# verlab/accelerated_features

Measured on NVIDIA B200. Metric: image-pairs/sec (extract+match) VGA batch=64, higher is better.
Workload: dtype f32

## Files before the change

### accelerated_features_b200/_lib.py

```python
from __future__ import annotations

import ctypes as C
import os

_HERE = os.path.dirname(os.path.abspath(__file__))
LIB_PATH = os.path.join(_HERE, "libxfeat_sm100.so")
_lib = None
ABI_VERSION = 2
N_OVERFLOW = -1

c_i, c_f, c_p, c_sz, c_i64 = C.c_int, C.c_float, C.c_void_p, C.c_size_t, C.c_int64

SIGNATURES = {
    "xfeat_abi_version": (c_i, []),
    "xfeat_last_error": (C.c_char_p, []),
    "xfeat_launch_count": (C.c_ulonglong, []),
    "xfeat_packed_weight_floats": (c_sz, []),
    "xfeat_create": (c_i, [C.POINTER(c_p), c_i, c_p, c_sz]),
    "xfeat_destroy": (None, [c_p]),
    "xfeat_resize_bilinear": (c_i, [c_p, c_i, c_i, c_i, c_i, c_i, c_i64, c_i64, c_i64, c_i64, c_i, c_p, c_i, c_i, c_f, c_f, c_p]),
    "xfeat_preprocess": (c_i, [c_p, c_i, c_i, c_i, c_i, c_i, c_i64, c_i64, c_i64, c_i64, c_i, c_i, c_i, c_p, c_p, c_p]),
    "xfeat_preprocess_scaled": (c_i, [c_p, c_i, c_i, c_i, c_i, c_i, c_i64, c_i64, c_i64, c_i64, c_i, c_i, c_i, c_f, c_f, c_p, c_p, c_p]),
    "xfeat_set_conv_impl": (None, [c_i]),
    "xfeat_set_halo_desc_mode": (None, [c_i]),
    "xfeat_get_conv_impl": (c_i, []),
    "xfeat_set_block1_fused": (None, [c_i]),
    "xfeat_get_block1_fused": (c_i, []),
    "xfeat_net_workspace_bytes": (c_sz, [c_i, c_i, c_i]),
    "xfeat_net": (c_i, [c_p, c_p, c_i, c_i, c_i, c_p, c_p, c_p, c_p, c_p, c_sz, c_p]),
    "xfeat_sparse_workspace_bytes": (c_sz, [c_i, c_i, c_i, c_i]),
    "xfeat_detect_sparse": (c_i, [c_p, c_p, c_p, c_p, c_i, c_i, c_i, c_i, c_f, c_f, c_f, c_p, c_p, c_p, c_p, c_p, c_p, c_p, c_sz, c_p]),
    "xfeat_detect_sparse_split": (c_i, [c_p, c_p, c_p, c_p, c_i, c_i, c_i, c_i, c_f, c_f, c_f, c_p, c_p, c_p, c_p, c_p, c_p, c_p, c_i, c_p, c_sz, c_p]),
    "xfeat_dense_workspace_bytes": (c_sz, [c_i, c_i, c_i, c_i]),
    "xfeat_detect_dense": (c_i, [c_p, c_p, c_p, c_i, c_i, c_i, c_i, c_f, c_f, c_f, c_f, c_i, c_i, c_p, c_p, c_p, c_p, c_p, c_sz, c_p]),
    "xfeat_set_mnn_impl": (None, [c_i]),
    "xfeat_get_mnn_impl": (c_i, []),
    "xfeat_mnn_workspace_bytes": (c_sz, [c_i, c_i, c_i]),
    "xfeat_mnn_match": (c_i, [c_p, c_p, c_i, c_i64, c_p, c_p, c_i, c_i64, c_i, c_f, c_p, c_p, c_p, c_p, c_sz, c_p]),
    "xfeat_mnn_match_bounded": (c_i, [c_p, c_p, c_i, c_i64, c_p, c_p, c_i, c_i64, c_i, c_f, c_f, c_p, c_p, c_p, c_p, c_sz, c_p]),
    "xfeat_mnn_presplit_workspace_bytes": (c_sz, [c_i, c_i, c_i]),
    "xfeat_mnn_match_presplit": (c_i, [c_p, c_p, c_i, c_p, c_p, c_i, c_i, c_i, c_i, c_f, c_p, c_p, c_p, c_p, c_sz, c_p]),
    "xfeat_gather_matches": (c_i, [c_p, c_p, c_i, c_i, c_p, c_p, c_p, c_i, c_p, c_p, c_p]),
    "xfeat_refine_workspace_bytes": (c_sz, [c_i, c_i]),
    "xfeat_refine": (c_i, [c_p, c_p, c_p, c_p, c_p, c_p, c_p, c_p, c_p, c_i, c_i, c_i, c_f, c_p, c_p, c_p, c_sz, c_p]),
    "xfeat_kpts_heatmap": (c_i, [c_p, c_i, c_i, c_i, c_f, c_p, c_p]),
    "xfeat_nms_workspace_bytes": (c_sz, [c_i, c_i, c_i]),
    "xfeat_nms_count": (c_i, [c_p, c_i, c_i, c_i, c_i, c_f, c_p, c_p, c_sz, c_p]),
    "xfeat_nms_write": (c_i, [c_p, c_i, c_i, c_i, c_i, c_f, c_p, c_i, c_p, c_sz, c_p]),
    "xfeat_interpolate_sparse": (c_i, [c_p, c_p, c_i, c_i, c_i, c_i, c_i, c_i, c_i, c_i, c_p, c_p]),
    "xfeat_subpix_softmax2d": (c_i, [c_p, c_i64, c_f, c_p, c_p]),
    "xfeat_fine_matcher_workspace_bytes": (c_sz, [c_i]),
    "xfeat_fine_matcher": (c_i, [c_p, c_p, c_i, c_p, c_p, c_sz, c_p]),
    "xfeat_ransac_workspace_bytes": (c_sz, [c_i, c_i]),
    "xfeat_ransac_homography": (c_i, [c_p, c_p, c_p, c_i, c_i, c_f, c_i, C.c_uint32, c_p, c_p, c_p, c_p, c_sz, c_p]),
    "xfeat_ransac_essential": (c_i, [c_p, c_p, c_p, c_i, c_i, c_f, c_i, C.c_uint32, c_p, c_p, c_p, c_p, c_sz, c_p]),
    "xfeat_debug_conv_layer": (c_i, [c_p, c_i, c_p, c_i, c_i, c_i, c_p, c_p]),
    "xfeat_debug_conv_layer_tc": (c_i, [c_p, c_i, c_p, c_i, c_i, c_i, c_p, c_p, c_sz, c_p]),
    "xfeat_debug_block1_tail": (c_i, [c_p, c_p, c_p, c_i, c_i, c_i, c_p, c_p, c_sz, c_p]),
}


class XFeatLibraryError(RuntimeError):
    pass


def load():
    global _lib
    if _lib is not None:
        return _lib
    if not os.path.exists(LIB_PATH):
        raise XFeatLibraryError(
            f"{LIB_PATH} not found: build it with `python -m accelerated_features_b200.build` "
            "(there is no CPU / PyTorch fallback for the XFeat hot path)")
    lib = C.CDLL(LIB_PATH)
    for name, (res, args) in SIGNATURES.items():
        fn = getattr(lib, name)
        fn.restype = res
        fn.argtypes = args
    if lib.xfeat_abi_version() != ABI_VERSION:
        raise XFeatLibraryError(f"ABI version mismatch: library {lib.xfeat_abi_version()} != binding {ABI_VERSION}")
    _lib = lib
    return lib


def check(rc: int, what: str = ""):
    if rc != 0:
        msg = load().xfeat_last_error().decode(errors="replace")
        raise XFeatLibraryError(f"{what} failed (code {rc}): {msg}")
```

### accelerated_features_b200/csrc/api.cu

```cuda
#include <stdarg.h>

#include <map>
#include <mutex>
#include <utility>
#include <vector>

#include "common.cuh"

namespace xf {

static thread_local char g_err[1024] = "";
unsigned long long g_launches = 0;
int g_conv_impl = 2;

int ensure_dyn_smem(const void* func, size_t bytes) {
  static std::mutex mu;
  static std::map<std::pair<int, const void*>, size_t> done;
  int dev = 0;
  XF_CUDA(cudaGetDevice(&dev));
  std::lock_guard<std::mutex> lock(mu);
  size_t& cur = done[std::make_pair(dev, func)];
  if (bytes > cur) {
    XF_CUDA(cudaFuncSetAttribute(func, cudaFuncAttributeMaxDynamicSharedMemorySize, (int)bytes));
    cur = bytes;
  }
  return XF_OK;
}

void set_error(const char* fmt, ...) {
  va_list ap;
  va_start(ap, fmt);
  vsnprintf(g_err, sizeof(g_err), fmt, ap);
  va_end(ap);
}

struct NetWs {
  float *a1, *a2, *a3, *x1s, *t4a, *x2;
  float *t8a, *t8b, *x3, *fin, *f1, *f2;
  float *t16a, *t16b, *x4;
  float *t32a, *t32b, *x5;
};

static void carve_net(Bump& bump, int B, int H, int W, NetWs& ws) {
  const size_t p1 = (size_t)B * H * W, p2 = p1 / 4, p4 = p1 / 16, p8 = p1 / 64, p16 = p1 / 256, p32 = p1 / 1024;
  ws.a1 = bump.take<float>(p1 * 4);
  ws.a2 = bump.take<float>(p2 * 8);
  ws.a3 = bump.take<float>(p2 * 8);
  ws.x1s = bump.take<float>(p4 * 32);
  ws.t4a = bump.take<float>(p4 * 32);
  ws.x2 = bump.take<float>(p4 * 32);
  ws.t8a = bump.take<float>(p8 * 64);
  ws.t8b = bump.take<float>(p8 * 64);
  ws.x3 = bump.take<float>(p8 * 64);
  ws.fin = bump.take<float>(p8 * 64);
  ws.f1 = bump.take<float>(p8 * 64);
  ws.f2 = bump.take<float>(p8 * 64);
  ws.t16a = bump.take<float>(p16 * 64);
  ws.t16b = bump.take<float>(p16 * 64);
  ws.x4 = bump.take<float>(p16 * 64);
  ws.t32a = bump.take<float>(p32 * 128);
  ws.t32b = bump.take<float>(p32 * 128);
  ws.x5 = bump.take<float>(p32 * 64);
}

}

extern "C" int xfeat_abi_version(void) { return XFEAT_ABI_VERSION; }
extern "C" const char* xfeat_last_error(void) { return xf::g_err; }
extern "C" unsigned long long xfeat_launch_count(void) { return xf::g_launches; }
extern "C" size_t xfeat_packed_weight_floats(void) { return xf::make_layer_table().total; }

extern "C" int xfeat_create(xfeat_ctx** out, int device, const float* packed_host, size_t n_floats) {
  XF_REQUIRE(out && packed_host, "create: null pointer");
  const xf::LayerTable t = xf::make_layer_table();
  XF_REQUIRE(n_floats == t.total, "create: packed blob has %zu floats, expected %zu", n_floats, t.total);
  xf::DeviceGuard guard(device);
  XF_REQUIRE(guard.ok, "create: cudaSetDevice(%d) failed", device);
  cudaDeviceProp prop;
  XF_CUDA(cudaGetDeviceProperties(&prop, device));
  if (prop.major != 10) {
    xf::set_error("create: device %d is sm_%d%d; this library contains sm_100a code only", device, prop.major, prop.minor);
    return XF_E_UNSUPPORTED;
  }
  xfeat_ctx* c = new xfeat_ctx();
  c->device = device;
  c->sm_count = prop.multiProcessorCount;
  c->table = t;
  c->h_weights = (float*)malloc(sizeof(float) * t.total);
  memcpy(c->h_weights, packed_host, sizeof(float) * t.total);
  c->d_weights = nullptr;
  cudaError_t e = cudaMalloc(&c->d_weights, sizeof(float) * t.total);
  if (e == cudaSuccess) e = cudaMemcpy(c->d_weights, packed_host, sizeof(float) * t.total, cudaMemcpyHostToDevice);
  if (e != cudaSuccess) {
    xf::set_error("create: weight upload failed: %s", cudaGetErrorString(e));
    if (c->d_weights) cudaFree(c->d_weights);
    free(c->h_weights);
    delete c;
    return XF_E_CUDA;
  }
  c->d_tcw = nullptr;
  c->d_mlpw = nullptr;
  int rc = xf::conv_tc_prepare(c);
  if (rc == XF_OK) rc = xf::mlp_tc_prepare(c);
  if (rc != XF_OK) {
    cudaFree(c->d_weights);
    if (c->d_tcw) cudaFree(c->d_tcw);
    if (c->d_mlpw) cudaFree(c->d_mlpw);
    free(c->h_weights);
    delete c;
    return rc;
  }
  *out = c;
  return XF_OK;
}

extern "C" void xfeat_set_conv_impl(int impl) { xf::g_conv_impl = (impl < 0 || impl > 2) ? 1 : impl; }
extern "C" int xfeat_get_conv_impl(void) { return xf::g_conv_impl; }

extern "C" void xfeat_destroy(xfeat_ctx* ctx) {
  if (!ctx) return;
  xf::DeviceGuard guard(ctx->device);
  if (ctx->d_weights) cudaFree(ctx->d_weights);
  if (ctx->d_tcw) cudaFree(ctx->d_tcw);
  if (ctx->d_mlpw) cudaFree(ctx->d_mlpw);
  free(ctx->h_weights);
  delete ctx;
}

extern "C" size_t xfeat_net_workspace_bytes(int B, int H, int W) {
  xf::Bump bump(nullptr, 0);
  xf::NetWs ws;
  xf::carve_net(bump, B, H, W, ws);
  return bump.used();
}

extern "C" int xfeat_net(xfeat_ctx* ctx, const float* d_xn, int B, int H, int W, float* d_feats, float* d_heat,
                         float* d_reliability, float* d_kpt_logits, void* d_ws, size_t ws_bytes, void* stream) {
  using namespace xf;
  XF_REQUIRE(ctx && d_xn && d_feats && d_heat && d_reliability && d_ws, "net: null pointer");
  XF_REQUIRE(B > 0 && B <= 65535 && H > 0 && W > 0 && H % 32 == 0 && W % 32 == 0, "net: bad shape B=%d H=%d W=%d", B, H, W);
  XF_CUDA(cudaSetDevice(ctx->device));
  cudaStream_t st = (cudaStream_t)stream;
  Bump bump(d_ws, ws_bytes);
  NetWs ws;
  carve_net(bump, B, H, W, ws);
  if (!bump.ok) {
    set_error("net: workspace too small (%zu < %zu)", ws_bytes, bump.used());
    return XF_E_WORKSPACE;
  }
  const int H4 = H / 4, W4 = W / 4, H8 = H / 8, W8 = W / 8, H16 = H / 16, W16 = W / 16, H32 = H / 32, W32 = W / 32;
  int rc;
#define XF_RUN(call) \
  if ((rc = (call)) != XF_OK) return rc
  if (g_conv_impl == 0) {
    XF_RUN(launch_stem_chain(ctx->h_weights, ctx->table, d_xn, ws.a1, ws.a2, ws.a3, ws.x1s, nullptr, B, H, W, st));
    XF_RUN(launch_conv_layer(ctx, L_B2_0, ws.x1s, IN_NHWC, B, H4, W4, ws.t4a, st));
    XF_RUN(launch_conv_layer(ctx, L_B2_1, ws.t4a, IN_NHWC, B, H4, W4, ws.x2, st));
    XF_RUN(launch_conv_layer(ctx, L_B3_0, ws.x2, IN_NHWC, B, H4, W4, ws.t8a, st));
    XF_RUN(launch_conv_layer(ctx, L_B3_1, ws.t8a, IN_NHWC, B, H8, W8, ws.t8b, st));
    XF_RUN(launch_conv_layer(ctx, L_B3_2, ws.t8b, IN_NHWC, B, H8, W8, ws.x3, st));
    XF_RUN(launch_conv_layer(ctx, L_B4_0, ws.x3, IN_NHWC, B, H8, W8, ws.t16a, st));
    XF_RUN(launch_conv_layer(ctx, L_B4_1, ws.t16a, IN_NHWC, B, H16, W16, ws.t16b, st));
    XF_RUN(launch_conv_layer(ctx, L_B4_2, ws.t16b, IN_NHWC, B, H16, W16, ws.x4, st));
    XF_RUN(launch_conv_layer(ctx, L_B5_0, ws.x4, IN_NHWC, B, H16, W16, ws.t32a, st));
  } else {
    __half *s4a = (__half*)ws.x1s, *s4b = (__half*)ws.t4a, *s4c = (__half*)ws.x2;
    __half *s8a = (__half*)ws.t8a, *s8b = (__half*)ws.t8b, *s16a = (__half*)ws.t16a, *s16b = (__half*)ws.t16b;
    if (g_conv_impl == 2) {
      XF_RUN(launch_stem_chain(ctx->h_weights, ctx->table, d_xn, ws.a1, ws.a2, ws.a3, nullptr, nullptr, B, H, W, st, 1));
      XF_RUN(launch_block1_tail(ctx, (const __half*)ws.a2, d_xn, B, H4, W4, (__half*)ws.a3, s4a, nullptr, st));
    } else {
      XF_RUN(launch_stem_chain(ctx->h_weights, ctx->table, d_xn, ws.a1, ws.a2, ws.a3, nullptr, s4a, B, H, W, st));
    }
    XF_RUN(launch_conv_tc(ctx, L_B2_0, s4a, B, H4, W4, s4b, nullptr, st));
    XF_RUN(launch_conv_tc(ctx, L_B2_1, s4b, B, H4, W4, s4c, nullptr, st));
    XF_RUN(launch_conv_tc(ctx, L_B3_0, s4c, B, H4, W4, s8a, nullptr, st));
    XF_RUN(launch_conv_tc(ctx, L_B3_1, s8a, B, H8, W8, s8b, nullptr, st));
    XF_RUN(launch_conv_tc(ctx, L_B3_2, s8b, B, H8, W8, s8a, nullptr, st));
    XF_RUN(launch_conv_tc(ctx, L_B4_0, s8a, B, H8, W8, s16a, nullptr, st));
    XF_RUN(launch_conv_tc(ctx, L_B4_1, s16a, B, H16, W16, s16b, nullptr, st));
    XF_RUN(launch_conv_tc(ctx, L_B4_2, s16b, B, H16, W16, s16a, nullptr, st));
    __half *s32a = (__half*)ws.t32a, *s32b = (__half*)ws.t32b;
    XF_RUN(launch_conv_tc(ctx, L_B5_0, s16a, B, H16, W16, s32a, nullptr, st));
    XF_RUN(launch_conv_tc(ctx, L_B5_1, s32a, B, H32, W32, s32b, nullptr, st));
    XF_RUN(launch_conv_tc(ctx, L_B5_2, s32b, B, H32, W32, s32a, nullptr, st));
    XF_RUN(launch_conv_tc(ctx, L_B5_3, s32a, B, H32, W32, s32b, nullptr, st));
  }
  if (g_conv_impl == 0) {
    XF_RUN(launch_conv_layer(ctx, L_B5_1, ws.t32a, IN_NHWC, B, H32, W32, ws.t32b, st));
    XF_RUN(launch_conv_layer(ctx, L_B5_2, ws.t32b, IN_NHWC, B, H32, W32, ws.t32a, st));
    XF_RUN(launch_conv_layer(ctx, L_B5_3, ws.t32a, IN_NHWC, B, H32, W32, ws.x5, st));
  }
  if (g_conv_impl == 0) {
    XF_RUN(launch_fuse_pyramid(ws.x3, ws.x4, ws.x5, ws.fin, nullptr, B, H8, W8, st));
    XF_RUN(launch_conv_layer(ctx, L_FU_0, ws.fin, IN_NHWC, B, H8, W8, ws.f1, st));
    XF_RUN(launch_conv_layer(ctx, L_FU_1, ws.f1, IN_NHWC, B, H8, W8, ws.f2, st));
    XF_RUN(launch_conv_layer(ctx, L_FU_2, ws.f2, IN_NHWC, B, H8, W8, d_feats, st));
    XF_RUN(launch_conv_layer(ctx, L_HH_0, d_feats, IN_NHWC, B, H8, W8, ws.t8a, st));
    XF_RUN(launch_conv_layer(ctx, L_HH_1, ws.t8a, IN_NHWC, B, H8, W8, ws.t8b, st));
    XF_RUN(launch_reliability(ctx, ws.t8b, d_reliability, (int64_t)B * H8 * W8, st));
    XF_RUN(launch_conv_layer(ctx, L_KH_0, d_xn, IN_UNFOLD8, B, H8, W8, ws.t8a, st));
    XF_RUN(launch_conv_layer(ctx, L_KH_1, ws.t8a, IN_NHWC, B, H8, W8, ws.t8b, st));
    XF_RUN(launch_conv_layer(ctx, L_KH_2, ws.t8b, IN_NHWC, B, H8, W8, ws.t8a, st));
    XF_RUN(launch_kpt_softmax(ctx, ws.t8a, d_heat, d_kpt_logits, B, H8, W8, st));
  } else {
    __half *s8a = (__half*)ws.t8a, *s8b = (__half*)ws.t8b, *sfin = (__half*)ws.fin, *sf1 = (__half*)ws.f1, *sf2 = (__half*)ws.f2;
    XF_RUN(launch_fuse_pyramid_split(s8a, (const __half*)ws.t16a, (const __half*)ws.t32b, sfin, B, H8, W8, st));
    XF_RUN(launch_conv_tc(ctx, L_FU_0, sfin, B, H8, W8, sf1, nullptr, st));
    XF_RUN(launch_conv_tc(ctx, L_FU_1, sf1, B, H8, W8, sf2, nullptr, st));
    XF_RUN(launch_conv_tc(ctx, L_FU_2, sf2, B, H8, W8, s8a, d_feats, st));
    if (g_conv_impl == 2) {
      XF_RUN(launch_head_chain(ctx, 1, s8a, B, H8, W8, d_reliability, nullptr, st));
      XF_RUN(launch_head_chain(ctx, 0, d_xn, B, H8, W8, d_heat, d_kpt_logits, st));
      return XF_OK;
    }
    XF_RUN(launch_conv_tc(ctx, L_HH_0, s8a, B, H8, W8, s8b, nullptr, st));
    XF_RUN(launch_conv_tc(ctx, L_HH_1, s8b, B, H8, W8, nullptr, ws.t8a, st));
    XF_RUN(launch_reliability(ctx, ws.t8a, d_reliability, (int64_t)B * H8 * W8, st));
    XF_RUN(launch_unfold8_split(d_xn, s8b, B, H8, W8, st));
    XF_RUN(launch_conv_tc(ctx, L_KH_0, s8b, B, H8, W8, s8a, nullptr, st));
    XF_RUN(launch_conv_tc(ctx, L_KH_1, s8a, B, H8, W8, s8b, nullptr, st));
    XF_RUN(launch_conv_tc(ctx, L_KH_2, s8b, B, H8, W8, nullptr, ws.t8a, st));
    XF_RUN(launch_kpt_softmax(ctx, ws.t8a, d_heat, d_kpt_logits, B, H8, W8, st));
  }
#undef XF_RUN
  return XF_OK;
}
```

### accelerated_features_b200/csrc/block1_tc.cu

```cuda
#include <cuda_fp16.h>

#include <stdlib.h>

#include "common.cuh"
#include "tc_common.cuh"

namespace xf {

constexpr int B1_THREADS = 448;
constexpr int B1_NP = 4;
constexpr int B1_W2_BYTES = 9 * 2 * 8 * 32;
constexpr int B1_W3_BYTES = 9 * 2 * 32 * 32;
constexpr int B1_W_PAD = 23 * 1024;
constexpr int B1_PB_MAX = 30 * 1024;
constexpr int B1_PLANE_MAX = 6 * 1024;

struct Block1Params {
  CUtensorMap amap;
  CUtensorMap w2map;
  CUtensorMap w3map;
  const float* bias2;
  const float* bias3;
  const float* skip_w;
  const float* xn;
  float inv_ws2, inv_ws3;
  int B, H4, W4;
  int TQH, TQW, PW2, PQW, M2;
  int PB, PLB;
  int tmem_cols;
  __half* out_split;
  float* out_f32;
  FastDiv div_img, div_x;
};

__global__ void __launch_bounds__(B1_THREADS, 1) block1_tc_kernel(const __grid_constant__ Block1Params P) {
  extern __shared__ unsigned char smem_raw[];
  unsigned char* base = reinterpret_cast<unsigned char*>(((uintptr_t)smem_raw + 1023) & ~(uintptr_t)1023);
  unsigned char* sW2 = base;
  unsigned char* sW3 = sW2 + B1_W2_BYTES;
  unsigned char* sP = base + B1_W_PAD;
  unsigned char* sQ = sP + (size_t)B1_NP * P.PB;
  uint64_t* bars = reinterpret_cast<uint64_t*>(sQ + (size_t)8 * P.PLB);
  uint64_t* w_full = bars;
  uint64_t* p_full = bars + 1;
  uint64_t* p_empty = p_full + B1_NP;
  uint64_t* acc2_full = p_empty + B1_NP;
  uint64_t* acc2_empty = acc2_full + 2;
  uint64_t* q_full = acc2_empty + 2;
  uint64_t* q_empty = q_full + 2;
  uint64_t* acc3_full = q_empty + 2;
  uint64_t* acc3_empty = acc3_full + 2;
  uint32_t* tmem_slot = reinterpret_cast<uint32_t*>(acc3_empty + 2);
  float* sB2 = reinterpret_cast<float*>(tmem_slot + 2);
  float* sB3 = sB2 + 8;
  float* sSkip = sB3 + 32;

  const int warp = threadIdx.x >> 5, lane = threadIdx.x & 31;
  const int tiles_x = (P.W4 + P.TQW - 1) / P.TQW, tiles_y = (P.H4 + P.TQH - 1) / P.TQH;
  const int tiles_img = tiles_x * tiles_y;
  const int n_tiles = tiles_img * P.B;
  const int H2 = 2 * P.H4, W2 = 2 * P.W4;
  const int ACC2 = P.M2 * 16;
  const uint32_t acc3_col = 2u * ACC2;

  if (threadIdx.x < 8) sB2[threadIdx.x] = __ldg(P.bias2 + threadIdx.x);
  if (threadIdx.x < 32) sB3[threadIdx.x] = threadIdx.x < 24 ? __ldg(P.bias3 + threadIdx.x) : 0.f;
  if (threadIdx.x < 64) {
    const int c = threadIdx.x % 32, wb = threadIdx.x / 32;
    sSkip[threadIdx.x] = c < 24 ? __ldg(P.skip_w + wb * 24 + c) : 0.f;
  }
  if (warp == 0 && lane == 0) {
    tc::tma_prefetch_desc(&P.amap);
    tc::tma_prefetch_desc(&P.w2map);
    tc::tma_prefetch_desc(&P.w3map);
    tc::mbar_init(w_full, 1);
    for (int i = 0; i < B1_NP; ++i) {
      tc::mbar_init(&p_full[i], 1);
      tc::mbar_init(&p_empty[i], 1);
    }
    for (int i = 0; i < 2; ++i) {
      tc::mbar_init(&acc2_full[i], 1);
      tc::mbar_init(&acc2_empty[i], 8);
      tc::mbar_init(&q_full[i], 8);
      tc::mbar_init(&q_empty[i], 1);
      tc::mbar_init(&acc3_full[i], 1);
      tc::mbar_init(&acc3_empty[i], 4);
    }
    tc::fence_barrier_init();
  }
  if (warp == 1) {
    tc::tmem_alloc(tmem_slot, P.tmem_cols);
    tc::tmem_relinquish();
  }
  tc::tc_fence_before();
  __syncthreads();
  tc::tc_fence_after();
  const uint32_t tmem = *tmem_slot;

  if (warp == 0) {
    if (tc::elect_one()) {
      tc::mbar_expect_tx(w_full, (uint32_t)(B1_W2_BYTES + B1_W3_BYTES));
      for (int i = 0; i < 18; ++i) tc::tma_load_2d(sW2 + i * 256, &P.w2map, w_full, 0, i * 8);
      for (int i = 0; i < 18; ++i) tc::tma_load_2d(sW3 + i * 1024, &P.w3map, w_full, 0, i * 32);
      const uint32_t patch_tx = (uint32_t)(2 * P.TQH + 3) * P.PW2 * 32;
      uint32_t tcount = 0;
      for (int tile = blockIdx.x; tile < n_tiles; tile += gridDim.x, ++tcount) {
        const int b = (int)fdiv((unsigned)tile, P.div_img), rem = tile - b * tiles_img;
        const int ty_ = (int)fdiv((unsigned)rem, P.div_x), tx_ = rem - ty_ * tiles_x;
        const int s = tcount % B1_NP;
        tc::mbar_wait(&p_empty[s], ((tcount / B1_NP) & 1) ^ 1);
        tc::mbar_expect_tx(&p_full[s], patch_tx);
        tc::tma_load_4d(sP + (size_t)s * P.PB, &P.amap, &p_full[s], 0, 2 * tx_ * P.TQW - 2, 2 * ty_ * P.TQH - 2, b);
      }
    }
    __syncwarp();
  } else if (warp == 1) {
    if (tc::elect_one()) {
      constexpr uint32_t idesc2 = tc::make_idesc( 0, 128, 16);
      constexpr uint32_t idesc3 = tc::make_idesc( 0, 128, 64);
      tc::mbar_wait(w_full, 0);
      const uint32_t w2_base = tc::smem_u32(sW2), w3_base = tc::smem_u32(sW3);
      const uint32_t p_base = tc::smem_u32(sP), q_base = tc::smem_u32(sQ);
      const int n_mine = n_tiles > (int)blockIdx.x ? (n_tiles - 1 - (int)blockIdx.x) / (int)gridDim.x + 1 : 0;
      for (int t = 0; t <= n_mine; ++t) {
        if (t < n_mine) {
          const int s = t % B1_NP, a = t & 1;
          tc::mbar_wait(&acc2_empty[a], ((t >> 1) & 1) ^ 1);
          tc::mbar_wait(&p_full[s], (t / B1_NP) & 1);
          tc::tc_fence_after();
          const uint32_t pb = p_base + (uint32_t)s * P.PB;
          for (int mt = 0; mt < P.M2; ++mt) {
            const uint32_t d = tmem + (uint32_t)(a * ACC2 + mt * 16);
            for (int tap = 0; tap < 9; ++tap) {
              const uint32_t row = (uint32_t)(mt * 128 + (tap / 3) * P.PW2 + (tap % 3));
              tc::umma_f16(d, tc::make_desc_sw32(pb + row * 32u, 256), tc::make_desc_sw32(w2_base + tap * 512u, 256), idesc2,
                           tap ? 1u : 0u);
            }
          }
          tc::umma_commit(&p_empty[s]);
          tc::umma_commit(&acc2_full[a]);
        }
        if (t > 0) {
          const int u = t - 1, a = u & 1;
          tc::mbar_wait(&acc3_empty[a], ((u >> 1) & 1) ^ 1);
          tc::mbar_wait(&q_full[a], (u >> 1) & 1);
          tc::tc_fence_after();
          const uint32_t qb = q_base + (uint32_t)a * 4u * P.PLB;
          const uint32_t d = tmem + acc3_col + (uint32_t)a * 64u;
          for (int tap = 0; tap < 9; ++tap) {
            const int ky = tap / 3, kx = tap % 3;
            const uint32_t addr = qb + (uint32_t)((ky & 1) * 2 + (kx & 1)) * P.PLB + (uint32_t)((ky >> 1) * P.PQW + (kx >> 1)) * 32u;
            tc::umma_f16(d, tc::make_desc_sw32(addr, 256), tc::make_desc_sw32(w3_base + tap * 2048u, 256), idesc3, tap ? 1u : 0u);
          }
          tc::umma_commit(&q_empty[a]);
          tc::umma_commit(&acc3_full[a]);
        }
      }
    }
    __syncwarp();
  } else if (warp < 10) {
    const int q = warp & 3, eg = (warp - 2) >> 2;
    const int hmax = 2 * P.TQH + 1, wmax = 2 * P.TQW + 1;
    uint32_t tcount = 0;
    for (int tile = blockIdx.x; tile < n_tiles; tile += gridDim.x, ++tcount) {
      const int a = tcount & 1;
      const int b = (int)fdiv((unsigned)tile, P.div_img), rem = tile - b * tiles_img;
      const int ty_ = (int)fdiv((unsigned)rem, P.div_x), tx_ = rem - ty_ * tiles_x;
      const int y0 = 2 * ty_ * P.TQH - 1, x0 = 2 * tx_ * P.TQW - 1;
      unsigned char* qb = sQ + (size_t)a * 4 * P.PLB;
      tc::mbar_wait(&acc2_full[a], (tcount >> 1) & 1);
      tc::mbar_wait(&q_empty[a], ((tcount >> 1) & 1) ^ 1);
      tc::tc_fence_after();
      for (int mt = eg; mt < P.M2; mt += 2) {
        uint32_t v[16];
        __syncwarp();
        tc::tmem_ld_32x16(tmem + ((uint32_t)(q * 32) << 16) + (uint32_t)(a * ACC2 + mt * 16), v);
        tc::tmem_ld_wait();
        const int m = mt * 128 + q * 32 + lane;
        const int h = m / P.PW2, w = m - h * P.PW2;
        if (h < hmax && w < wmax) {
          const int y = y0 + h, x = x0 + w;
          uint32_t hw[4] = {0u, 0u, 0u, 0u}, lw[4] = {0u, 0u, 0u, 0u};
          if (y >= 0 && y < H2 && x >= 0 && x < W2) {
            float o[8];
#pragma unroll
            for (int c = 0; c < 8; ++c) o[c] = fmaxf(fmaf(__uint_as_float(v[c]) + __uint_as_float(v[8 + c]), P.inv_ws2, sB2[c]), 0.f);
#pragma unroll
            for (int j = 0; j < 4; ++j) {
              const __half2 hh = __floats2half2_rn(o[2 * j], o[2 * j + 1]);
              const float2 hf = __half22float2(hh);
              const __half2 ll = __floats2half2_rn(o[2 * j] - hf.x, o[2 * j + 1] - hf.y);
              hw[j] = *reinterpret_cast<const uint32_t*>(&hh);
              lw[j] = *reinterpret_cast<const uint32_t*>(&ll);
            }
          }
          const int r = (h >> 1) * P.PQW + (w >> 1);
          unsigned char* rp = qb + (size_t)((h & 1) * 2 + (w & 1)) * P.PLB + r * 32;
          const int sw = (r >> 2) & 1;
          *reinterpret_cast<uint4*>(rp + (sw << 4)) = make_uint4(hw[0], hw[1], hw[2], hw[3]);
          *reinterpret_cast<uint4*>(rp + ((sw ^ 1) << 4)) = make_uint4(lw[0], lw[1], lw[2], lw[3]);
        }
      }
      tc::fence_proxy_async();
      tc::tc_fence_before();
      __syncwarp();
      if (lane == 0) {
        tc::mbar_arrive(&acc2_empty[a]);
        tc::mbar_arrive(&q_full[a]);
      }
    }
  } else {
    const int q = warp & 3;
    const int m = q * 32 + lane;
    const int i = m / P.PQW, j = m - i * P.PQW;
    const bool lane_ok = (i < P.TQH) && (j < P.TQW);
    const int W0 = P.W4 * 4;
    auto fetch_xn = [&](int tile, float4 (&xv)[4]) {
      if (tile >= n_tiles) return;
      const int b = (int)fdiv((unsigned)tile, P.div_img), rem = tile - b * tiles_img;
      const int ty_ = (int)fdiv((unsigned)rem, P.div_x), tx_ = rem - ty_ * tiles_x;
      const int y = ty_ * P.TQH + i, x = tx_ * P.TQW + j;
      if (lane_ok && y < P.H4 && x < P.W4) {
        const float* xp = P.xn + ((int64_t)b * P.H4 * 4 + y * 4) * W0 + x * 4;
#pragma unroll
        for (int rr = 0; rr < 4; ++rr) xv[rr] = __ldg(reinterpret_cast<const float4*>(xp + (int64_t)rr * W0));
      }
    };
    float4 xv[4] = {};
    fetch_xn(blockIdx.x, xv);
    uint32_t tcount = 0;
    for (int tile = blockIdx.x; tile < n_tiles; tile += gridDim.x, ++tcount) {
      const int a = tcount & 1;
      const int b = (int)fdiv((unsigned)tile, P.div_img), rem = tile - b * tiles_img;
      const int ty_ = (int)fdiv((unsigned)rem, P.div_x), tx_ = rem - ty_ * tiles_x;
      const int y = ty_ * P.TQH + i, x = tx_ * P.TQW + j;
      float4 xnext[4] = {};
      fetch_xn(tile + (int)gridDim.x, xnext);
      tc::mbar_wait(&acc3_full[a], (tcount >> 1) & 1);
      tc::tc_fence_after();
      uint32_t v[64];
      __syncwarp();
#pragma unroll
      for (int c = 0; c < 2; ++c) {
        uint32_t t[32];
        tc::tmem_ld_32x32(tmem + ((uint32_t)(q * 32) << 16) + acc3_col + (uint32_t)a * 64u + c * 32, t);
#pragma unroll
        for (int k = 0; k < 32; ++k) v[c * 32 + k] = t[k];
      }
      tc::tmem_ld_wait();
      tc::tc_fence_before();
      __syncwarp();
      if (lane == 0) tc::mbar_arrive(&acc3_empty[a]);
      if (lane_ok && y < P.H4 && x < P.W4) {
        const int64_t pix = ((int64_t)b * P.H4 + y) * P.W4 + x;
        float o[32];
#pragma unroll
        for (int c = 0; c < 32; ++c) o[c] = fmaxf(fmaf(__uint_as_float(v[c]) + __uint_as_float(v[32 + c]), P.inv_ws3, sB3[c]), 0.f);
        float sacc = 0.f;
#pragma unroll
        for (int rr = 0; rr < 4; ++rr) {
          sacc += xv[rr].x; sacc += xv[rr].y; sacc += xv[rr].z; sacc += xv[rr].w;
        }
        const float skipv = sacc * (1.0f / 16.0f);
#pragma unroll
        for (int c = 0; c < 32; ++c) o[c] += fmaf(skipv, sSkip[c], sSkip[32 + c]);
        if (P.out_f32) tc::store_f32_row<32>(P.out_f32 + pix * 24, o, 24);
        if (P.out_split) {
          __half* hp = P.out_split + pix * 64;
          tc::store_split_row<32>(hp, hp + 32, o);
        }
      }
#pragma unroll
      for (int rr = 0; rr < 4; ++rr) xv[rr] = xnext[rr];
    }
  }
  tc::tc_fence_before();
  __syncthreads();
  if (warp == 1) {
    tc::tc_fence_after();
    tc::tmem_dealloc(tmem, P.tmem_cols);
  }
}

struct Block1Tile { int TQH, TQW, M2; };

static Block1Tile pick_block1_tile(int H4, int W4) {
  Block1Tile best = {0, 0, 0};
  double best_cost = 1e30;
  for (int tqw = 4; tqw <= 62; ++tqw) {
    const int pqw = tqw + 1, pw2 = 2 * tqw + 3;
    for (int tqh = 1; tqh * pqw <= 128; ++tqh) {
      const int m2 = cdiv((2 * tqh + 1) * pw2, 128);
      if ((m2 * 128 + 2 * pw2 + 2) * 32 > B1_PB_MAX || (128 + pqw + 1) * 32 > B1_PLANE_MAX) continue;
      const double tiles = (double)cdiv(W4, tqw) * cdiv(H4, tqh);
      const double cost = tiles * ((m2 + 1) * 128.0 + 0.15 * (2 * tqh + 3) * pw2);
      if (cost < best_cost) { best_cost = cost; best = {tqh, tqw, m2}; }
    }
  }
  return best;
}

int g_block1_fused = 1;

static bool block1_fused() {
  static const bool unfused = getenv("XFEAT_BLOCK1_UNFUSED") != nullptr;
  return g_block1_fused && !unfused;
}

static int launch_block1_fused(const xfeat_ctx* ctx, const __half* a2_split, const float* xn, int B, int H4, int W4,
                               __half* out_split, float* out_f32, cudaStream_t st) {
  PFN_encodeTiled enc = get_encode_tiled();
  if (!enc) {
    set_error("cuTensorMapEncodeTiled entry point not available");
    return XF_E_CUDA;
  }
  const Block1Tile tl = pick_block1_tile(H4, W4);
  Block1Params P;
  P.TQH = tl.TQH; P.TQW = tl.TQW; P.M2 = tl.M2;
  P.PW2 = 2 * tl.TQW + 3;
  P.PQW = tl.TQW + 1;
  P.PB = (int)align_up((size_t)(tl.M2 * 128 + 2 * P.PW2 + 2) * 32, 1024);
  P.PLB = (int)align_up((size_t)(128 + P.PQW + 1) * 32, 1024);
  int cols = 32;
  while (cols < 2 * tl.M2 * 16 + 128) cols *= 2;
  P.tmem_cols = cols;
  const int H2 = 2 * H4, W2 = 2 * W4;
  const cuuint64_t dims[4] = {16, (cuuint64_t)W2, (cuuint64_t)H2, (cuuint64_t)B};
  const cuuint64_t strides[3] = {32, (cuuint64_t)W2 * 32, (cuuint64_t)H2 * W2 * 32};
  const cuuint32_t box[4] = {16, (cuuint32_t)P.PW2, (cuuint32_t)(2 * P.TQH + 3), 1};
  const cuuint32_t estr[4] = {1, 1, 1, 1};
  CUresult r = enc(&P.amap, CU_TENSOR_MAP_DATA_TYPE_FLOAT16, 4, (void*)a2_split, dims, strides, box, estr,
                   CU_TENSOR_MAP_INTERLEAVE_NONE, CU_TENSOR_MAP_SWIZZLE_32B, CU_TENSOR_MAP_L2_PROMOTION_L2_256B,
                   CU_TENSOR_MAP_FLOAT_OOB_FILL_NONE);
  if (r != CUDA_SUCCESS) {
    set_error("cuTensorMapEncodeTiled(block1 a2 patch) failed: %d", (int)r);
    return XF_E_CUDA;
  }
  const int layers[2] = {L_B1_2, L_B1_3}, nrows[2] = {8, 32};
  CUtensorMap* maps[2] = {&P.w2map, &P.w3map};
  for (int k = 0; k < 2; ++k) {
    const cuuint64_t wdims[2] = {16, (cuuint64_t)18 * nrows[k]};
    const cuuint64_t wstrides[1] = {32};
    const cuuint32_t wbox[2] = {16, (cuuint32_t)nrows[k]};
    const cuuint32_t westr[2] = {1, 1};
    r = enc(maps[k], CU_TENSOR_MAP_DATA_TYPE_FLOAT16, 2, (void*)((__half*)ctx->d_tcw + ctx->tc_off[layers[k]]), wdims, wstrides,
            wbox, westr, CU_TENSOR_MAP_INTERLEAVE_NONE, CU_TENSOR_MAP_SWIZZLE_32B, CU_TENSOR_MAP_L2_PROMOTION_L2_256B,
            CU_TENSOR_MAP_FLOAT_OOB_FILL_NONE);
    if (r != CUDA_SUCCESS) {
      set_error("cuTensorMapEncodeTiled(block1 weights, layer %d) failed: %d", layers[k], (int)r);
      return XF_E_CUDA;
    }
  }
  P.bias2 = ctx->d_weights + ctx->table.b_off[L_B1_2];
  P.bias3 = ctx->d_weights + ctx->table.b_off[L_B1_3];
  P.skip_w = ctx->d_weights + ctx->table.w_off[L_SKIP1];
  P.xn = xn;
  P.inv_ws2 = ctx->tc_inv_wscale[L_B1_2];
  P.inv_ws3 = ctx->tc_inv_wscale[L_B1_3];
  P.B = B; P.H4 = H4; P.W4 = W4;
  P.out_split = out_split;
  P.out_f32 = out_f32;
  const int tiles_img = cdiv(H4, P.TQH) * cdiv(W4, P.TQW);
  const int n_tiles = tiles_img * B;
  XF_REQUIRE(n_tiles < (1 << 22), "block1_tc: too many tiles (%d)", n_tiles);
  P.div_img = make_fastdiv((unsigned)tiles_img);
  P.div_x = make_fastdiv((unsigned)cdiv(W4, P.TQW));
  const size_t smem = 1024 + B1_W_PAD + (size_t)B1_NP * P.PB + (size_t)8 * P.PLB + 1024;
  const int grid = n_tiles < ctx->sm_count ? n_tiles : ctx->sm_count;
  XF_DYN_SMEM(block1_tc_kernel, smem);
  block1_tc_kernel<<<grid, B1_THREADS, smem, st>>>(P);
  XF_LAUNCH_CHECK();
  return XF_OK;
}

int launch_block1_tail(const xfeat_ctx* ctx, const __half* a2_split, const float* xn, int B, int H4, int W4, __half* a3_split,
                       __half* out_split, float* out_f32, cudaStream_t st) {
  XF_REQUIRE(ctx->d_tcw && ctx->tc_off[L_B1_2] != (size_t)-1 && ctx->tc_off[L_B1_3] != (size_t)-1,
             "block1_tc: block1 weights not prepared for the tensor-core path");
  XF_REQUIRE(out_split || out_f32, "block1_tc: no output");
  if (block1_fused()) return launch_block1_fused(ctx, a2_split, xn, B, H4, W4, out_split, out_f32, st);
  int rc = launch_conv_tc(ctx, L_B1_2, a2_split, B, 2 * H4, 2 * W4, a3_split, nullptr, st);
  if (rc) return rc;
  return launch_conv_tc(ctx, L_B1_3, a3_split, B, 2 * H4, 2 * W4, out_split, out_f32, st, xn);
}

}

extern "C" void xfeat_set_block1_fused(int on) { xf::g_block1_fused = on ? 1 : 0; }
extern "C" int xfeat_get_block1_fused(void) { return xf::block1_fused() ? 1 : 0; }

extern "C" int xfeat_debug_block1_tail(xfeat_ctx* ctx, const float* d_a2, const float* d_xn, int B, int H, int W, float* d_x1s,
                                       void* d_scratch, size_t scratch_bytes, void* stream) {
  XF_REQUIRE(ctx && d_a2 && d_xn && d_x1s && d_scratch, "debug_block1_tail: null pointer");
  XF_REQUIRE(B > 0 && B <= 65535 && H > 0 && W > 0 && H % 4 == 0 && W % 4 == 0, "debug_block1_tail: bad shape B=%d H=%d W=%d", B,
             H, W);
  const int64_t npix2 = (int64_t)B * (H / 2) * (W / 2);
  XF_REQUIRE(scratch_bytes >= (size_t)npix2 * 64, "debug_block1_tail: scratch must hold B*(H/2)*(W/2)*64 bytes");
  XF_CUDA(cudaSetDevice(ctx->device));
  cudaStream_t st = (cudaStream_t)stream;
  __half* a2s = (__half*)d_scratch;
  int rc = xf::launch_split_nhwc(d_a2, a2s, npix2, 8, 8, st);
  if (rc) return rc;
  return xf::launch_block1_tail(ctx, a2s, d_xn, B, H / 4, W / 4, a2s + npix2 * 16, nullptr, d_x1s, st);
}
```

### accelerated_features_b200/csrc/common.cuh

```cuda
#pragma once
#include <cuda.h>
#include <cuda_fp16.h>
#include <cuda_runtime.h>
#include <stdint.h>
#include <stdio.h>
#include <string>

#include "../../include/xfeat_b200.h"
#include "layers.h"

namespace xf {

void set_error(const char* fmt, ...);


#define XF_CUDA(expr)                                                                      \
  do {                                                                                     \
    cudaError_t _e = (expr);                                                               \
    if (_e != cudaSuccess) {                                                               \
      xf::set_error("%s:%d: %s -> %s", __FILE__, __LINE__, #expr, cudaGetErrorString(_e)); \
      return XF_E_CUDA;                                                                    \
    }                                                                                      \
  } while (0)

extern unsigned long long g_launches;
#define XF_LAUNCH_CHECK()          \
  do {                             \
    ++xf::g_launches;              \
    XF_CUDA(cudaGetLastError());   \
  } while (0)

#define XF_REQUIRE(cond, ...)       \
  do {                              \
    if (!(cond)) {                  \
      xf::set_error(__VA_ARGS__);   \
      return XF_E_INVALID;          \
    }                               \
  } while (0)

int ensure_dyn_smem(const void* func, size_t bytes);
#define XF_DYN_SMEM(kernel, bytes)                                                   \
  do {                                                                               \
    int _rc = xf::ensure_dyn_smem((const void*)(kernel), (size_t)(bytes));           \
    if (_rc != XF_OK) return _rc;                                                    \
  } while (0)

struct DeviceGuard {
  int prev;
  bool ok;
  explicit DeviceGuard(int dev) : prev(-1), ok(false) {
    if (cudaGetDevice(&prev) != cudaSuccess) prev = -1;
    ok = (cudaSetDevice(dev) == cudaSuccess);
  }
  ~DeviceGuard() {
    if (prev >= 0) cudaSetDevice(prev);
  }
};

static inline int cdiv(int a, int b) { return (a + b - 1) / b; }
static inline size_t align_up(size_t x, size_t a) { return (x + a - 1) / a * a; }

struct Bump {
  char* base;
  size_t off, cap;
  bool ok;
  Bump(void* p, size_t bytes) : base((char*)p), off(0), cap(bytes), ok(true) {}
  template <typename T>
  T* take(size_t n) {
    off = align_up(off, 256);
    size_t b = n * sizeof(T);
    if (base != nullptr && off + b > cap) ok = false;
    T* r = base ? (T*)(base + off) : nullptr;
    off += b;
    return r;
  }
  size_t used() const { return align_up(off, 256); }
};

__host__ __device__ __forceinline__ uint32_t f2ord(float f) {
#ifdef __CUDA_ARCH__
  uint32_t u = __float_as_uint(f);
#else
  uint32_t u;
  memcpy(&u, &f, 4);
#endif
  return (u & 0x80000000u) ? ~u : (u | 0x80000000u);
}
__host__ __device__ __forceinline__ float ord2f(uint32_t o) {
  uint32_t u = (o & 0x80000000u) ? (o & 0x7fffffffu) : ~o;
#ifdef __CUDA_ARCH__
  return __uint_as_float(u);
#else
  float f;
  memcpy(&f, &u, 4);
  return f;
#endif
}
__device__ __forceinline__ unsigned long long pack_vi(float v, uint32_t idx) {
  return ((unsigned long long)f2ord(v + 0.0f) << 32) | (unsigned long long)(0xffffffffu - idx);
}
__device__ __forceinline__ uint32_t packed_idx(unsigned long long p) { return 0xffffffffu - (uint32_t)(p & 0xffffffffu); }
__device__ __forceinline__ float packed_val(unsigned long long p) { return ord2f((uint32_t)(p >> 32)); }

__device__ __forceinline__ float sparse_src_coord(int p, int size_pos, int size_map) {
  float g = __fsub_rn(__fmul_rn(2.0f, __fdiv_rn((float)p, (float)(size_pos - 1))), 1.0f);
  return __fdiv_rn(__fsub_rn(__fmul_rn(__fadd_rn(g, 1.0f), (float)size_map), 1.0f), 2.0f);
}

__device__ __forceinline__ float2 f2_fma(float2 a, float2 b, float2 c) {
  float2 r;
  asm("fma.rn.f32x2 %0, %1, %2, %3;"
      : "=l"(*reinterpret_cast<unsigned long long*>(&r))
      : "l"(*reinterpret_cast<const unsigned long long*>(&a)), "l"(*reinterpret_cast<const unsigned long long*>(&b)),
        "l"(*reinterpret_cast<const unsigned long long*>(&c)));
  return r;
}
__device__ __forceinline__ float2 f2_mul(float2 a, float2 b) {
  float2 r;
  asm("mul.rn.f32x2 %0, %1, %2;"
      : "=l"(*reinterpret_cast<unsigned long long*>(&r))
      : "l"(*reinterpret_cast<const unsigned long long*>(&a)), "l"(*reinterpret_cast<const unsigned long long*>(&b)));
  return r;
}

struct LinTap {
  int i0, i1;
  float l0, l1;
};
__device__ __forceinline__ LinTap lin_tap(int dst, float scale, int in_size) {
  float src = __fsub_rn(__fmul_rn(scale, __fadd_rn((float)dst, 0.5f)), 0.5f);
  if (src < 0.f) src = 0.f;
  LinTap t;
  t.i0 = (int)src;
  if (t.i0 > in_size - 1) t.i0 = in_size - 1;
  t.i1 = t.i0 + ((t.i0 < in_size - 1) ? 1 : 0);
  t.l1 = __fsub_rn(src, (float)t.i0);
  t.l0 = __fsub_rn(1.0f, t.l1);
  return t;
}

}

struct xfeat_ctx {
  int device;
  int sm_count;
  float* d_weights;
  float* h_weights;
  xf::LayerTable table;
  void* d_tcw;
  size_t tc_off[xf::L_COUNT];
  float tc_inv_wscale[xf::L_COUNT];
  void* d_mlpw;
  size_t mlp_off[5];
  float mlp_inv_scale[5];
};

namespace xf {
enum { IN_NHWC = 0, IN_UNFOLD8 = 1 };
int launch_conv_layer(const xfeat_ctx* ctx, int layer, const float* in, int in_mode, int B, int Hi, int Wi,
                      float* out, cudaStream_t st, const int* n_live = nullptr, __half* out_split = nullptr);
extern int g_conv_impl;
bool conv_tc_eligible(int layer);
int launch_conv_tc_halo(const xfeat_ctx* ctx, int layer, const __half* in_split, int B, int H, int W, __half* out_split,
                        float* out_f32, cudaStream_t st);
int launch_topk_select_sort(const unsigned long long* keys, const int* n_keep, int n_const, int cap, int top_k, int B,
                            unsigned long long* sorted, cudaStream_t st);
int conv_tc_prepare(xfeat_ctx* ctx);
int mlp_tc_prepare(xfeat_ctx* ctx);
int launch_fine_mlp_tc(const xfeat_ctx* ctx, const __half* X_split, int rows_cap, const int* n_live, __half* act_a, __half* act_b,
                       float* logits, cudaStream_t st);
int launch_conv_tc(const xfeat_ctx* ctx, int layer, const __half* in_split, int B, int H, int W, __half* out_split,
                   float* out_f32, cudaStream_t st, const float* skip_xn = nullptr);
int launch_block1_tail(const xfeat_ctx* ctx, const __half* a2_split, const float* xn, int B, int H4, int W4, __half* a3_split,
                       __half* out_split, float* out_f32, cudaStream_t st);
int launch_head_chain(const xfeat_ctx* ctx, int mode, const void* in, int B, int Hc, int Wc, float* out, float* logits,
                      cudaStream_t st);
int launch_split_nhwc(const float* in, __half* out, int64_t npix, int C, int CP, cudaStream_t st);
int launch_unfold8_split(const float* xn, __half* out, int B, int Hc, int Wc, cudaStream_t st);
int launch_stem_chain(const float* h_weights, const LayerTable& t, const float* xn, float* a1, float* a2, float* a3,
                      float* x1s, __half* x1s_split32, int B, int H, int W, cudaStream_t st, int tc_tail = 0);
int launch_fuse_pyramid(const float* x3, const float* x4, const float* x5, float* out, __half* out_split, int B, int H3,
                        int W3, cudaStream_t st);
int launch_fuse_pyramid_split(const __half* x3, const __half* x4, const __half* x5, __half* out_split, int B, int H3, int W3,
                              cudaStream_t st);
int launch_reliability(const xfeat_ctx* ctx, const float* t, float* out, int64_t npix, cudaStream_t st);
int launch_kpt_softmax(const xfeat_ctx* ctx, const float* t, float* heat, float* logits, int B, int Hc, int Wc,
                       cudaStream_t st);
}
```

### accelerated_features_b200/csrc/stem.cu

```cuda
#include "common.cuh"

namespace xf {

template <int CIN, int COUT>
struct StemW {
  float w[9 * CIN * COUT];
  float b[COUT];
};
struct SkipW {
  float w[24];
  float b[24];
};

template <int CIN>
__device__ __forceinline__ void load_vec(const float* __restrict__ p, float (&v)[CIN]) {
  if constexpr (CIN == 1) {
    v[0] = __ldg(p);
  } else {
#pragma unroll
    for (int i = 0; i < CIN / 4; ++i) {
      const float4 t = __ldg(reinterpret_cast<const float4*>(p) + i);
      v[4 * i + 0] = t.x; v[4 * i + 1] = t.y; v[4 * i + 2] = t.z; v[4 * i + 3] = t.w;
    }
  }
}

template <int CIN, int COUT, int S, bool SKIP>
__global__ void __launch_bounds__(128) stem_conv_kernel(const __grid_constant__ StemW<CIN, COUT> P,
                                                        const __grid_constant__ SkipW K,
                                                        const float* __restrict__ in, const float* __restrict__ xn,
                                                        float* __restrict__ out, __half* __restrict__ out_split32, int Hi,
                                                        int Wi, int Ho, int Wo) {
  const int ox = blockIdx.x * 32 + (threadIdx.x & 31);
  const int oy = blockIdx.y * 4 + (threadIdx.x >> 5);
  const int b = blockIdx.z;
  if (ox >= Wo || oy >= Ho) return;
  float acc[COUT];
#pragma unroll
  for (int co = 0; co < COUT; ++co) acc[co] = 0.f;
  const float* inb = in + (int64_t)b * Hi * Wi * CIN;
#pragma unroll
  for (int ky = 0; ky < 3; ++ky) {
    const int iy = oy * S - 1 + ky;
#pragma unroll
    for (int kx = 0; kx < 3; ++kx) {
      const int ix = ox * S - 1 + kx;
      float v[CIN];
      if (iy >= 0 && iy < Hi && ix >= 0 && ix < Wi) {
        load_vec<CIN>(inb + ((int64_t)iy * Wi + ix) * CIN, v);
      } else {
#pragma unroll
        for (int ci = 0; ci < CIN; ++ci) v[ci] = 0.f;
      }
#pragma unroll
      for (int ci = 0; ci < CIN; ++ci)
#pragma unroll
        for (int co = 0; co < COUT; ++co)
          acc[co] = fmaf(v[ci], P.w[((ky * 3 + kx) * CIN + ci) * COUT + co], acc[co]);
    }
  }
  float skipv = 0.f;
  if constexpr (SKIP) {
    const int W0 = Wo * 4;
    const float* xp = xn + ((int64_t)b * Ho * 4 + oy * 4) * W0 + ox * 4;
    float s = 0.f;
#pragma unroll
    for (int r = 0; r < 4; ++r) {
      const float4 t = __ldg(reinterpret_cast<const float4*>(xp + (int64_t)r * W0));
      s += t.x; s += t.y; s += t.z; s += t.w;
    }
    skipv = s * (1.0f / 16.0f);
  }
  float res[COUT];
#pragma unroll
  for (int co = 0; co < COUT; ++co) {
    float v = fmaxf(acc[co] + P.b[co], 0.f);
    if constexpr (SKIP) v += fmaf(skipv, K.w[co], K.b[co]);
    res[co] = v;
  }
  if constexpr (COUT == 24) {
    if (out_split32 != nullptr) {
      uint4* sp = reinterpret_cast<uint4*>(out_split32 + (((int64_t)b * Ho + oy) * Wo + ox) * 64);
#pragma unroll
      for (int g = 0; g < 4; ++g) {
        uint32_t hw[4], lw[4];
#pragma unroll
        for (int j = 0; j < 4; ++j) {
          const int c = 8 * g + 2 * j;
          const float x0 = (c < 24) ? res[c < 24 ? c : 0] : 0.f, x1 = (c + 1 < 24) ? res[c + 1 < 24 ? c + 1 : 0] : 0.f;
          const __half2 h = __floats2half2_rn(x0, x1);
          const float2 hf = __half22float2(h);
          const __half2 l = __floats2half2_rn(x0 - hf.x, x1 - hf.y);
          hw[j] = *reinterpret_cast<const uint32_t*>(&h);
          lw[j] = *reinterpret_cast<const uint32_t*>(&l);
        }
        sp[g] = make_uint4(hw[0], hw[1], hw[2], hw[3]);
        sp[4 + g] = make_uint4(lw[0], lw[1], lw[2], lw[3]);
      }
      return;
    }
  }
  if constexpr (COUT == 8) {
    if (out_split32 != nullptr) {
      uint32_t hw[4], lw[4];
#pragma unroll
      for (int j = 0; j < 4; ++j) {
        const __half2 h = __floats2half2_rn(res[2 * j], res[2 * j + 1]);
        const float2 hf = __half22float2(h);
        const __half2 l = __floats2half2_rn(res[2 * j] - hf.x, res[2 * j + 1] - hf.y);
        hw[j] = *reinterpret_cast<const uint32_t*>(&h);
        lw[j] = *reinterpret_cast<const uint32_t*>(&l);
      }
      uint4* sp = reinterpret_cast<uint4*>(out_split32 + (((int64_t)b * Ho + oy) * Wo + ox) * 16);
      sp[0] = make_uint4(hw[0], hw[1], hw[2], hw[3]);
      sp[1] = make_uint4(lw[0], lw[1], lw[2], lw[3]);
      return;
    }
  }
  float* op = out + (((int64_t)b * Ho + oy) * Wo + ox) * COUT;
#pragma unroll
  for (int c4 = 0; c4 < COUT / 4; ++c4)
    reinterpret_cast<float4*>(op)[c4] = make_float4(res[4 * c4], res[4 * c4 + 1], res[4 * c4 + 2], res[4 * c4 + 3]);
}

template <int CIN, int COUT, int S, bool SKIP>
static int launch_stem(const float* hw, const float* hb, const float* sw, const float* sb, const float* in,
                       const float* xn, float* out, __half* out_split32, int B, int Hi, int Wi, cudaStream_t st) {
  StemW<CIN, COUT> P;
  memcpy(P.w, hw, sizeof(P.w));
  memcpy(P.b, hb, sizeof(P.b));
  SkipW K;
  memset(&K, 0, sizeof(K));
  if (SKIP) { memcpy(K.w, sw, sizeof(K.w)); memcpy(K.b, sb, sizeof(K.b)); }
  const int Ho = Hi / S, Wo = Wi / S;
  dim3 grid(cdiv(Wo, 32), cdiv(Ho, 4), B);
  stem_conv_kernel<CIN, COUT, S, SKIP><<<grid, 128, 0, st>>>(P, K, in, xn, out, out_split32, Hi, Wi, Ho, Wo);
  XF_LAUNCH_CHECK();
  return XF_OK;
}

struct Stem01W {
  float w0[9 * 4];
  float b0[4];
  float w1[9 * 4 * 8];
  float b1[8];
};

__device__ __forceinline__ float2 fma2(float a, float2 w, float2 c) {
  float2 r;
  const float2 aa = make_float2(a, a);
  asm("fma.rn.f32x2 %0, %1, %2, %3;"
      : "=l"(*reinterpret_cast<unsigned long long*>(&r))
      : "l"(*reinterpret_cast<const unsigned long long*>(&aa)), "l"(*reinterpret_cast<const unsigned long long*>(&w)),
        "l"(*reinterpret_cast<const unsigned long long*>(&c)));
  return r;
}

__global__ void __launch_bounds__(128) stem01_kernel(const __grid_constant__ Stem01W P, const float* __restrict__ xn,
                                                     __half* __restrict__ out_split8, int H, int W) {
  const int Ho = H >> 1, Wo = W >> 1;
  const int ox0 = (blockIdx.x * 32 + (threadIdx.x & 31)) * 2;
  const int oy0 = (blockIdx.y * 4 + (threadIdx.x >> 5)) * 2;
  const int b = blockIdx.z;
  if (ox0 >= Wo || oy0 >= Ho) return;
  const float* xb = xn + (int64_t)b * H * W;
  const int gy0 = 2 * oy0 - 2, gx0 = 2 * ox0 - 2;
  float g[7][7];
#pragma unroll
  for (int r = 0; r < 7; ++r) {
    const int y = gy0 + r;
    const bool yin = y >= 0 && y < H;
    const float* row = xb + (int64_t)(yin ? y : 0) * W;
#pragma unroll
    for (int c = 0; c < 7; ++c) {
      const int x = gx0 + c;
      g[r][c] = (yin && x >= 0 && x < W) ? __ldg(row + x) : 0.f;
    }
  }
  float2 acc[2][2][4];
#pragma unroll
  for (int i = 0; i < 16; ++i) (&acc[0][0][0])[i] = make_float2(0.f, 0.f);
#pragma unroll
  for (int r = 0; r < 5; ++r) {
    const int ay = 2 * oy0 - 1 + r;
#pragma unroll
    for (int c = 0; c < 5; ++c) {
      const int ax = 2 * ox0 - 1 + c;
      float2 a2[2] = {make_float2(0.f, 0.f), make_float2(0.f, 0.f)};
#pragma unroll
      for (int ky = 0; ky < 3; ++ky)
#pragma unroll
        for (int kx = 0; kx < 3; ++kx) {
          const float gv = g[r + ky][c + kx];
          const float* w = &P.w0[(ky * 3 + kx) * 4];
          a2[0] = fma2(gv, make_float2(w[0], w[1]), a2[0]);
          a2[1] = fma2(gv, make_float2(w[2], w[3]), a2[1]);
        }
      const bool ain = ay >= 0 && ay < H && ax >= 0 && ax < W;
      float a[4] = {a2[0].x, a2[0].y, a2[1].x, a2[1].y};
#pragma unroll
      for (int ch = 0; ch < 4; ++ch) a[ch] = ain ? fmaxf(a[ch] + P.b0[ch], 0.f) : 0.f;
#pragma unroll
      for (int dy = 0; dy < 2; ++dy) {
        const int ky = r - 2 * dy;
        if (ky < 0 || ky > 2) continue;
#pragma unroll
        for (int dx = 0; dx < 2; ++dx) {
          const int kx = c - 2 * dx;
          if (kx < 0 || kx > 2) continue;
#pragma unroll
          for (int ci = 0; ci < 4; ++ci) {
            const float* w = &P.w1[((ky * 3 + kx) * 4 + ci) * 8];
#pragma unroll
            for (int cp = 0; cp < 4; ++cp) acc[dy][dx][cp] = fma2(a[ci], make_float2(w[2 * cp], w[2 * cp + 1]), acc[dy][dx][cp]);
          }
        }
      }
    }
  }
#pragma unroll
  for (int dy = 0; dy < 2; ++dy) {
    uint4* sp = reinterpret_cast<uint4*>(out_split8 + (((int64_t)b * Ho + oy0 + dy) * Wo + ox0) * 16);
#pragma unroll
    for (int dx = 0; dx < 2; ++dx) {
      uint32_t hw[4], lw[4];
#pragma unroll
      for (int j = 0; j < 4; ++j) {
        const float v0 = fmaxf(acc[dy][dx][j].x + P.b1[2 * j], 0.f), v1 = fmaxf(acc[dy][dx][j].y + P.b1[2 * j + 1], 0.f);
        const __half2 h = __floats2half2_rn(v0, v1);
        const float2 hf = __half22float2(h);
        const __half2 l = __floats2half2_rn(v0 - hf.x, v1 - hf.y);
        hw[j] = *reinterpret_cast<const uint32_t*>(&h);
        lw[j] = *reinterpret_cast<const uint32_t*>(&l);
      }
      sp[2 * dx] = make_uint4(hw[0], hw[1], hw[2], hw[3]);
      sp[2 * dx + 1] = make_uint4(lw[0], lw[1], lw[2], lw[3]);
    }
  }
}

static int g_stem_fused = 1;

int launch_stem_chain(const float* h_weights, const LayerTable& t, const float* xn, float* a1, float* a2, float* a3,
                      float* x1s, __half* x1s_split32, int B, int H, int W, cudaStream_t st, int tc_tail) {
  const float* hw = h_weights;
  int rc;
  static const bool unfused = getenv("XFEAT_STEM_UNFUSED") != nullptr;
  if (tc_tail && g_stem_fused && !unfused) {
    Stem01W P;
    memcpy(P.w0, hw + t.w_off[L_B1_0], sizeof(P.w0));
    memcpy(P.b0, hw + t.b_off[L_B1_0], sizeof(P.b0));
    memcpy(P.w1, hw + t.w_off[L_B1_1], sizeof(P.w1));
    memcpy(P.b1, hw + t.b_off[L_B1_1], sizeof(P.b1));
    dim3 grid(cdiv(W / 4, 32), cdiv(H / 4, 4), B);
    stem01_kernel<<<grid, 128, 0, st>>>(P, xn, (__half*)a2, H, W);
    XF_LAUNCH_CHECK();
    return XF_OK;
  }
  rc = launch_stem<1, 4, 1, false>(hw + t.w_off[L_B1_0], hw + t.b_off[L_B1_0], nullptr, nullptr, xn, nullptr, a1, nullptr, B, H, W, st);
  if (rc) return rc;
  rc = launch_stem<4, 8, 2, false>(hw + t.w_off[L_B1_1], hw + t.b_off[L_B1_1], nullptr, nullptr, a1, nullptr, a2,
                                   tc_tail ? (__half*)a2 : nullptr, B, H, W, st);
  if (rc || tc_tail) return rc;
  rc = launch_stem<8, 8, 1, false>(hw + t.w_off[L_B1_2], hw + t.b_off[L_B1_2], nullptr, nullptr, a2, nullptr, a3, nullptr, B, H / 2, W / 2, st);
  if (rc) return rc;
  rc = launch_stem<8, 24, 2, true>(hw + t.w_off[L_B1_3], hw + t.b_off[L_B1_3], hw + t.w_off[L_SKIP1], hw + t.b_off[L_SKIP1],
                                   a3, xn, x1s, x1s_split32, B, H / 2, W / 2, st);
  return rc;
}

}
```

### include/xfeat_b200.h

```cpp
#ifndef XFEAT_B200_H
#define XFEAT_B200_H

#include <stddef.h>
#include <stdint.h>

#ifdef __cplusplus
extern "C" {
#endif

#define XFEAT_ABI_VERSION 2
#if defined(__GNUC__)
#define XF_API __attribute__((visibility("default")))
#else
#define XF_API
#endif

enum {
  XF_OK = 0,
  XF_E_INVALID = 1,
  XF_E_CUDA = 2,
  XF_E_WORKSPACE = 3,
  XF_E_UNSUPPORTED = 4
};

#define XF_N_OVERFLOW (-1)

enum { XF_DTYPE_F32 = 0, XF_DTYPE_U8 = 1 };

typedef struct xfeat_ctx xfeat_ctx;

XF_API int xfeat_abi_version(void);
XF_API const char* xfeat_last_error(void);
XF_API unsigned long long xfeat_launch_count(void);

XF_API size_t xfeat_packed_weight_floats(void);

XF_API int xfeat_create(xfeat_ctx** out, int device, const float* packed_host, size_t n_floats);
XF_API void xfeat_destroy(xfeat_ctx* ctx);


XF_API int xfeat_resize_bilinear(const void* d_in, int dtype, int B, int C, int Hi, int Wi, int64_t stride_b,
                                 int64_t stride_c, int64_t stride_h, int64_t stride_w, int div255, float* d_out, int Ho,
                                 int Wo, float scale_h, float scale_w, void* stream);

XF_API int xfeat_preprocess(const void* d_img, int dtype, int B, int C, int Hi, int Wi,
                     int64_t stride_b, int64_t stride_c, int64_t stride_h, int64_t stride_w, int div255,
                     int H, int W, float* d_xn, double* d_stats, void* stream);

XF_API int xfeat_preprocess_scaled(const void* d_img, int dtype, int B, int C, int Hi, int Wi,
                            int64_t stride_b, int64_t stride_c, int64_t stride_h, int64_t stride_w, int div255,
                            int H, int W, float scale_h, float scale_w, float* d_xn, double* d_stats, void* stream);

XF_API void xfeat_set_halo_desc_mode(int mode);
XF_API void xfeat_set_conv_impl(int impl);
XF_API int xfeat_get_conv_impl(void);
XF_API void xfeat_set_block1_fused(int on);
XF_API int xfeat_get_block1_fused(void);
XF_API size_t xfeat_net_workspace_bytes(int B, int H, int W);
XF_API int xfeat_net(xfeat_ctx* ctx, const float* d_xn, int B, int H, int W, float* d_feats, float* d_heat,
              float* d_reliability, float* d_kpt_logits, void* d_ws, size_t ws_bytes, void* stream);

XF_API size_t xfeat_sparse_workspace_bytes(int B, int H, int W, int top_k);
XF_API int xfeat_detect_sparse(xfeat_ctx* ctx, const float* d_feats, const float* d_heat, const float* d_reliability,
                        int B, int H, int W, int top_k, float threshold, float rw, float rh,
                        float* d_kpts, float* d_scores, float* d_desc, int32_t* d_n_valid, int32_t* d_n_cand,
                        int32_t* d_kpts_int, void* d_ws, size_t ws_bytes, void* stream);

#define XF_DESC_SPLIT_SCALE_LOG2 13
XF_API int xfeat_detect_sparse_split(xfeat_ctx* ctx, const float* d_feats, const float* d_heat, const float* d_reliability,
                              int B, int H, int W, int top_k, float threshold, float rw, float rh, float* d_kpts,
                              float* d_scores, float* d_desc, int32_t* d_n_valid, int32_t* d_n_cand, int32_t* d_kpts_int,
                              void* d_desc_split, int split_rows, void* d_ws, size_t ws_bytes, void* stream);

XF_API size_t xfeat_dense_workspace_bytes(int B, int H, int W, int top_k);
XF_API int xfeat_detect_dense(xfeat_ctx* ctx, const float* d_feats, const float* d_reliability, int B, int H, int W,
                       int top_k, float rw, float rh, float div_scale, float scale_value, int out_rows, int out_offset,
                       float* d_kpts, float* d_desc, float* d_scales, int32_t* d_topk_idx, void* d_ws, size_t ws_bytes,
                       void* stream);

XF_API void xfeat_set_mnn_impl(int impl);
XF_API int xfeat_get_mnn_impl(void);
XF_API size_t xfeat_mnn_workspace_bytes(int batch, int n1_max, int n2_max);
XF_API int xfeat_mnn_match(const float* d_f1, const int32_t* d_n1, int n1_max, int64_t stride1,
                    const float* d_f2, const int32_t* d_n2, int n2_max, int64_t stride2,
                    int batch, float min_cossim, int64_t* d_idx0, int64_t* d_idx1, int32_t* d_n_matches,
                    void* d_ws, size_t ws_bytes, void* stream);
XF_API int xfeat_mnn_match_bounded(const float* d_f1, const int32_t* d_n1, int n1_max, int64_t stride1,
                            const float* d_f2, const int32_t* d_n2, int n2_max, int64_t stride2,
                            int batch, float min_cossim, float abs_bound, int64_t* d_idx0, int64_t* d_idx1,
                            int32_t* d_n_matches, void* d_ws, size_t ws_bytes, void* stream);

XF_API size_t xfeat_mnn_presplit_workspace_bytes(int batch, int n1_max, int n2_max);
XF_API int xfeat_mnn_match_presplit(const void* d_f1s, const int32_t* d_n1, int n1_max, const void* d_f2s, const int32_t* d_n2,
                             int n2_max, int n_pad, int batch, int scale_log2, float min_cossim, int64_t* d_idx0,
                             int64_t* d_idx1, int32_t* d_n_matches, void* d_ws, size_t ws_bytes, void* stream);

XF_API int xfeat_gather_matches(const float* d_kpts0, const float* d_kpts1, int n1_max, int n2_max,
                         const int64_t* d_idx0, const int64_t* d_idx1, const int32_t* d_n_matches, int batch,
                         float* d_out0, float* d_out1, void* stream);

XF_API size_t xfeat_refine_workspace_bytes(int batch, int n_max);
XF_API int xfeat_refine(xfeat_ctx* ctx, const float* d_desc0, const float* d_desc1, const float* d_kpts0,
                 const float* d_kpts1, const float* d_scales0, const int64_t* d_idx0, const int64_t* d_idx1,
                 const int32_t* d_n_matches, int batch, int n_max, int n1_max, float fine_conf, float* d_matches,
                 int32_t* d_n_refined, void* d_ws, size_t ws_bytes, void* stream);


XF_API int xfeat_kpts_heatmap(const float* d_logits, int B, int Hc, int Wc, float softmax_temp, float* d_heat, void* stream);

XF_API size_t xfeat_nms_workspace_bytes(int B, int H, int W);
XF_API int xfeat_nms_count(const float* d_heat, int B, int H, int W, int kernel_size, float threshold, int32_t* d_counts,
                           void* d_ws, size_t ws_bytes, void* stream);
XF_API int xfeat_nms_write(const float* d_heat, int B, int H, int W, int kernel_size, float threshold, int64_t* d_pos,
                           int pos_cap, void* d_ws, size_t ws_bytes, void* stream);

XF_API int xfeat_interpolate_sparse(const float* d_x, const float* d_pos, int B, int C, int Hm, int Wm, int N, int H, int W,
                                    int mode, float* d_out, void* stream);

XF_API int xfeat_subpix_softmax2d(const float* d_maps, int64_t n, float temp, float* d_out, void* stream);

XF_API size_t xfeat_fine_matcher_workspace_bytes(int n);
XF_API int xfeat_fine_matcher(xfeat_ctx* ctx, const float* d_x, int n, float* d_out, void* d_ws, size_t ws_bytes, void* stream);


XF_API size_t xfeat_ransac_workspace_bytes(int batch, int iters);
XF_API int xfeat_ransac_homography(const float* d_pts0, const float* d_pts1, const int32_t* d_n, int n_max, int batch,
                                   float thr_px, int iters, uint32_t seed, float* d_H, uint8_t* d_inliers,
                                   int32_t* d_n_inliers, void* d_ws, size_t ws_bytes, void* stream);

XF_API int xfeat_ransac_essential(const float* d_x0, const float* d_x1, const int32_t* d_n, int n_max, int batch, float thr,
                                  int iters, uint32_t seed, float* d_E, uint8_t* d_inliers, int32_t* d_n_inliers, void* d_ws,
                                  size_t ws_bytes, void* stream);

XF_API int xfeat_debug_conv_layer(xfeat_ctx* ctx, int layer, const float* d_in, int B, int Hi, int Wi, float* d_out,
                           void* stream);

XF_API int xfeat_debug_conv_layer_tc(xfeat_ctx* ctx, int layer, const float* d_in, int B, int H, int W, float* d_out,
                                     void* d_scratch, size_t scratch_bytes, void* stream);

XF_API int xfeat_debug_block1_tail(xfeat_ctx* ctx, const float* d_a2, const float* d_xn, int B, int H, int W, float* d_x1s,
                                   void* d_scratch, size_t scratch_bytes, void* stream);

#ifdef __cplusplus
}
#endif
#endif
```

Baseline: 20750.

## Fuse stem convolutions into block1 tensor-core kernel via dedicated producer warps

Adds a templated block1 kernel variant with eight extra producer warps. These warps cp.async the raw input tile into shared memory, compute the first two stem convolutions and the skip average on CUDA cores, and write the fp16 split patches straight into the MMA pipeline buffers. This removes the separate stem01 launch and its global round-trip of the a2 activation. The epilogue also now reads TMEM in 16-column halves to lower register pressure. In exchange, shared memory use grows, the block gets larger, and the producers' FP32 work may become the bottleneck for the tensor-core consumers.

New measurement: 14430, median of 6. -30.5%, worse.

```diff
diff --git a/accelerated_features_b200/_lib.py b/accelerated_features_b200/_lib.py
--- a/accelerated_features_b200/_lib.py
+++ b/accelerated_features_b200/_lib.py
@@ -26,6 +26,8 @@
     "xfeat_get_conv_impl": (c_i, []),
     "xfeat_set_block1_fused": (None, [c_i]),
     "xfeat_get_block1_fused": (c_i, []),
+    "xfeat_set_stem_fused": (None, [c_i]),
+    "xfeat_get_stem_fused": (c_i, []),
     "xfeat_net_workspace_bytes": (c_sz, [c_i, c_i, c_i]),
     "xfeat_net": (c_i, [c_p, c_p, c_i, c_i, c_i, c_p, c_p, c_p, c_p, c_p, c_sz, c_p]),
     "xfeat_sparse_workspace_bytes": (c_sz, [c_i, c_i, c_i, c_i]),
@@ -57,6 +59,7 @@
     "xfeat_debug_conv_layer": (c_i, [c_p, c_i, c_p, c_i, c_i, c_i, c_p, c_p]),
     "xfeat_debug_conv_layer_tc": (c_i, [c_p, c_i, c_p, c_i, c_i, c_i, c_p, c_p, c_sz, c_p]),
     "xfeat_debug_block1_tail": (c_i, [c_p, c_p, c_p, c_i, c_i, c_i, c_p, c_p, c_sz, c_p]),
+    "xfeat_debug_block1": (c_i, [c_p, c_p, c_i, c_i, c_i, c_p, c_p, c_sz, c_p]),
 }
 
 
diff --git a/accelerated_features_b200/csrc/api.cu b/accelerated_features_b200/csrc/api.cu
--- a/accelerated_features_b200/csrc/api.cu
+++ b/accelerated_features_b200/csrc/api.cu
@@ -167,8 +167,7 @@
     __half *s4a = (__half*)ws.x1s, *s4b = (__half*)ws.t4a, *s4c = (__half*)ws.x2;
     __half *s8a = (__half*)ws.t8a, *s8b = (__half*)ws.t8b, *s16a = (__half*)ws.t16a, *s16b = (__half*)ws.t16b;
     if (g_conv_impl == 2) {
-      XF_RUN(launch_stem_chain(ctx->h_weights, ctx->table, d_xn, ws.a1, ws.a2, ws.a3, nullptr, nullptr, B, H, W, st, 1));
-      XF_RUN(launch_block1_tail(ctx, (const __half*)ws.a2, d_xn, B, H4, W4, (__half*)ws.a3, s4a, nullptr, st));
+      XF_RUN(launch_block1(ctx, d_xn, B, H4, W4, (__half*)ws.a2, (__half*)ws.a3, s4a, nullptr, st));
     } else {
       XF_RUN(launch_stem_chain(ctx->h_weights, ctx->table, d_xn, ws.a1, ws.a2, ws.a3, nullptr, s4a, B, H, W, st));
     }
diff --git a/accelerated_features_b200/csrc/block1_tc.cu b/accelerated_features_b200/csrc/block1_tc.cu
--- a/accelerated_features_b200/csrc/block1_tc.cu
+++ b/accelerated_features_b200/csrc/block1_tc.cu
@@ -1,14 +1,20 @@
 #include <cuda_fp16.h>
 
 #include <stdlib.h>
+#include <type_traits>
 
 #include "common.cuh"
 #include "tc_common.cuh"
 
 namespace xf {
 
-constexpr int B1_THREADS = 448;
+constexpr int B1_BASE_WARPS = 14;
+constexpr int B1_PROD_WARPS = 8;
+template <bool FROM_XN>
+constexpr int b1_threads() { return 32 * (B1_BASE_WARPS + (FROM_XN ? B1_PROD_WARPS : 0)); }
 constexpr int B1_NP = 4;
+constexpr int B1_SKR = 8;
+constexpr int B1_SMEM_MAX = 227 * 1024;
 constexpr int B1_W2_BYTES = 9 * 2 * 8 * 32;
 constexpr int B1_W3_BYTES = 9 * 2 * 32 * 32;
 constexpr int B1_W_PAD = 23 * 1024;
@@ -28,19 +34,35 @@
   int TQH, TQW, PW2, PQW, M2;
   int PB, PLB;
   int tmem_cols;
+  Stem01W sw;
+  int XB, AB;
+  int XWP, AWP;
+  FastDiv div_xw, div_awp, div_pw2;
   __half* out_split;
   float* out_f32;
   FastDiv div_img, div_x;
 };
 
-__global__ void __launch_bounds__(B1_THREADS, 1) block1_tc_kernel(const __grid_constant__ Block1Params P) {
+__device__ __forceinline__ void cp_async4(void* smem_dst, const void* src, bool valid) {
+  asm volatile("cp.async.ca.shared.global [%0], [%1], 4, %2;" ::"r"(tc::smem_u32(smem_dst)), "l"(src), "r"(valid ? 4 : 0)
+               : "memory");
+}
+__device__ __forceinline__ void cp_async_commit() { asm volatile("cp.async.commit_group;" ::: "memory"); }
+__device__ __forceinline__ void cp_async_wait_all() { asm volatile("cp.async.wait_group 0;" ::: "memory"); }
+__device__ __forceinline__ uint32_t half2_bits(__half2 h) { return *reinterpret_cast<const uint32_t*>(&h); }
+
+template <bool FROM_XN>
+__global__ void __launch_bounds__(b1_threads<FROM_XN>(), 1) block1_tc_kernel(const __grid_constant__ Block1Params P) {
   extern __shared__ unsigned char smem_raw[];
   unsigned char* base = reinterpret_cast<unsigned char*>(((uintptr_t)smem_raw + 1023) & ~(uintptr_t)1023);
   unsigned char* sW2 = base;
   unsigned char* sW3 = sW2 + B1_W2_BYTES;
   unsigned char* sP = base + B1_W_PAD;
   unsigned char* sQ = sP + (size_t)B1_NP * P.PB;
-  uint64_t* bars = reinterpret_cast<uint64_t*>(sQ + (size_t)8 * P.PLB);
+  float* sX = reinterpret_cast<float*>(sQ + (size_t)8 * P.PLB);
+  float4* sA = reinterpret_cast<float4*>(reinterpret_cast<unsigned char*>(sX) + 2 * (size_t)P.XB);
+  float* sSk = reinterpret_cast<float*>(reinterpret_cast<unsigned char*>(sA) + P.AB);
+  uint64_t* bars = reinterpret_cast<uint64_t*>(sSk + (FROM_XN ? B1_SKR * 128 : 0));
   uint64_t* w_full = bars;
   uint64_t* p_full = bars + 1;
   uint64_t* p_empty = p_full + B1_NP;
@@ -50,7 +72,9 @@
   uint64_t* q_empty = q_full + 2;
   uint64_t* acc3_full = q_empty + 2;
   uint64_t* acc3_empty = acc3_full + 2;
-  uint32_t* tmem_slot = reinterpret_cast<uint32_t*>(acc3_empty + 2);
+  uint64_t* sk_full = acc3_empty + 2;
+  uint64_t* sk_empty = sk_full + B1_SKR;
+  uint32_t* tmem_slot = reinterpret_cast<uint32_t*>(sk_empty + B1_SKR);
   float* sB2 = reinterpret_cast<float*>(tmem_slot + 2);
   float* sB3 = sB2 + 8;
   float* sSkip = sB3 + 32;
@@ -70,12 +94,12 @@
     sSkip[threadIdx.x] = c < 24 ? __ldg(P.skip_w + wb * 24 + c) : 0.f;
   }
   if (warp == 0 && lane == 0) {
-    tc::tma_prefetch_desc(&P.amap);
+    if (!FROM_XN) tc::tma_prefetch_desc(&P.amap);
     tc::tma_prefetch_desc(&P.w2map);
     tc::tma_prefetch_desc(&P.w3map);
     tc::mbar_init(w_full, 1);
     for (int i = 0; i < B1_NP; ++i) {
-      tc::mbar_init(&p_full[i], 1);
+      tc::mbar_init(&p_full[i], FROM_XN ? B1_PROD_WARPS : 1);
       tc::mbar_init(&p_empty[i], 1);
     }
     for (int i = 0; i < 2; ++i) {
@@ -86,6 +110,10 @@
       tc::mbar_init(&acc3_full[i], 1);
       tc::mbar_init(&acc3_empty[i], 4);
     }
+    for (int i = 0; i < (FROM_XN ? B1_SKR : 0); ++i) {
+      tc::mbar_init(&sk_full[i], 4);
+      tc::mbar_init(&sk_empty[i], 4);
+    }
     tc::fence_barrier_init();
   }
   if (warp == 1) {
@@ -102,15 +130,17 @@
       tc::mbar_expect_tx(w_full, (uint32_t)(B1_W2_BYTES + B1_W3_BYTES));
       for (int i = 0; i < 18; ++i) tc::tma_load_2d(sW2 + i * 256, &P.w2map, w_full, 0, i * 8);
       for (int i = 0; i < 18; ++i) tc::tma_load_2d(sW3 + i * 1024, &P.w3map, w_full, 0, i * 32);
-      const uint32_t patch_tx = (uint32_t)(2 * P.TQH + 3) * P.PW2 * 32;
-      uint32_t tcount = 0;
-      for (int tile = blockIdx.x; tile < n_tiles; tile += gridDim.x, ++tcount) {
-        const int b = (int)fdiv((unsigned)tile, P.div_img), rem = tile - b * tiles_img;
-        const int ty_ = (int)fdiv((unsigned)rem, P.div_x), tx_ = rem - ty_ * tiles_x;
-        const int s = tcount % B1_NP;
-        tc::mbar_wait(&p_empty[s], ((tcount / B1_NP) & 1) ^ 1);
-        tc::mbar_expect_tx(&p_full[s], patch_tx);
-        tc::tma_load_4d(sP + (size_t)s * P.PB, &P.amap, &p_full[s], 0, 2 * tx_ * P.TQW - 2, 2 * ty_ * P.TQH - 2, b);
+      if constexpr (!FROM_XN) {
+        const uint32_t patch_tx = (uint32_t)(2 * P.TQH + 3) * P.PW2 * 32;
+        uint32_t tcount = 0;
+        for (int tile = blockIdx.x; tile < n_tiles; tile += gridDim.x, ++tcount) {
+          const int b = (int)fdiv((unsigned)tile, P.div_img), rem = tile - b * tiles_img;
+          const int ty_ = (int)fdiv((unsigned)rem, P.div_x), tx_ = rem - ty_ * tiles_x;
+          const int s = tcount % B1_NP;
+          tc::mbar_wait(&p_empty[s], ((tcount / B1_NP) & 1) ^ 1);
+          tc::mbar_expect_tx(&p_full[s], patch_tx);
+          tc::tma_load_4d(sP + (size_t)s * P.PB, &P.amap, &p_full[s], 0, 2 * tx_ * P.TQW - 2, 2 * ty_ * P.TQH - 2, b);
+        }
       }
     }
     __syncwarp();
@@ -209,7 +239,7 @@
         tc::mbar_arrive(&q_full[a]);
       }
     }
-  } else {
+  } else if (warp < B1_BASE_WARPS) {
     const int q = warp & 3;
     const int m = q * 32 + lane;
     const int i = m / P.PQW, j = m - i * P.PQW;
@@ -227,51 +257,195 @@
       }
     };
     float4 xv[4] = {};
-    fetch_xn(blockIdx.x, xv);
+    if (!FROM_XN) fetch_xn(blockIdx.x, xv);
     uint32_t tcount = 0;
     for (int tile = blockIdx.x; tile < n_tiles; tile += gridDim.x, ++tcount) {
       const int a = tcount & 1;
       const int b = (int)fdiv((unsigned)tile, P.div_img), rem = tile - b * tiles_img;
       const int ty_ = (int)fdiv((unsigned)rem, P.div_x), tx_ = rem - ty_ * tiles_x;
       const int y = ty_ * P.TQH + i, x = tx_ * P.TQW + j;
+      float skipv;
       float4 xnext[4] = {};
-      fetch_xn(tile + (int)gridDim.x, xnext);
+      if constexpr (FROM_XN) {
+        const int k = tcount % B1_SKR;
+        tc::mbar_wait(&sk_full[k], (tcount / B1_SKR) & 1);
+        skipv = sSk[k * 128 + m];
+        __syncwarp();
+        if (lane == 0) tc::mbar_arrive(&sk_empty[k]);
+      } else {
+        fetch_xn(tile + (int)gridDim.x, xnext);
+        float sacc = 0.f;
+#pragma unroll
+        for (int rr = 0; rr < 4; ++rr) {
+          sacc += xv[rr].x; sacc += xv[rr].y; sacc += xv[rr].z; sacc += xv[rr].w;
+        }
+        skipv = sacc * (1.0f / 16.0f);
+      }
       tc::mbar_wait(&acc3_full[a], (tcount >> 1) & 1);
       tc::tc_fence_after();
-      uint32_t v[64];
-      __syncwarp();
-#pragma unroll
-      for (int c = 0; c < 2; ++c) {
-        uint32_t t[32];
-        tc::tmem_ld_32x32(tmem + ((uint32_t)(q * 32) << 16) + acc3_col + (uint32_t)a * 64u + c * 32, t);
-#pragma unroll
-        for (int k = 0; k < 32; ++k) v[c * 32 + k] = t[k];
-      }
-      tc::tmem_ld_wait();
-      tc::tc_fence_before();
-      __syncwarp();
-      if (lane == 0) tc::mbar_arrive(&acc3_empty[a]);
-      if (lane_ok && y < P.H4 && x < P.W4) {
-        const int64_t pix = ((int64_t)b * P.H4 + y) * P.W4 + x;
-        float o[32];
-#pragma unroll
-        for (int c = 0; c < 32; ++c) o[c] = fmaxf(fmaf(__uint_as_float(v[c]) + __uint_as_float(v[32 + c]), P.inv_ws3, sB3[c]), 0.f);
-        float sacc = 0.f;
-#pragma unroll
-        for (int rr = 0; rr < 4; ++rr) {
-          sacc += xv[rr].x; sacc += xv[rr].y; sacc += xv[rr].z; sacc += xv[rr].w;
-        }
-        const float skipv = sacc * (1.0f / 16.0f);
-#pragma unroll
-        for (int c = 0; c < 32; ++c) o[c] += fmaf(skipv, sSkip[c], sSkip[32 + c]);
-        if (P.out_f32) tc::store_f32_row<32>(P.out_f32 + pix * 24, o, 24);
-        if (P.out_split) {
-          __half* hp = P.out_split + pix * 64;
-          tc::store_split_row<32>(hp, hp + 32, o);
-        }
-      }
-#pragma unroll
-      for (int rr = 0; rr < 4; ++rr) xv[rr] = xnext[rr];
+      const bool ok = lane_ok && y < P.H4 && x < P.W4;
+      const int64_t pix = ((int64_t)b * P.H4 + y) * P.W4 + x;
+      const uint32_t tacc = tmem + ((uint32_t)(q * 32) << 16) + acc3_col + (uint32_t)a * 64u;
+#pragma unroll
+      for (int hh = 0; hh < 2; ++hh) {
+        uint32_t vh[16], vl[16];
+        __syncwarp();
+        tc::tmem_ld_32x16(tacc + hh * 16, vh);
+        tc::tmem_ld_32x16(tacc + 32 + hh * 16, vl);
+        tc::tmem_ld_wait();
+        if (hh == 1) {
+          tc::tc_fence_before();
+          __syncwarp();
+          if (lane == 0) tc::mbar_arrive(&acc3_empty[a]);
+        }
+        if (ok) {
+          float o[16];
+#pragma unroll
+          for (int c = 0; c < 16; ++c) {
+            const int ch = hh * 16 + c;
+            o[c] = fmaxf(fmaf(__uint_as_float(vh[c]) + __uint_as_float(vl[c]), P.inv_ws3, sB3[ch]), 0.f);
+            o[c] += fmaf(skipv, sSkip[ch], sSkip[32 + ch]);
+          }
+          if (P.out_f32) tc::store_f32_row<16>(P.out_f32 + pix * 24 + hh * 16, o, hh ? 8 : 16);
+          if (P.out_split) {
+            __half* hp = P.out_split + pix * 64 + hh * 16;
+            tc::store_split_row<16>(hp, hp + 32, o);
+          }
+        }
+      }
+      if constexpr (!FROM_XN) {
+#pragma unroll
+        for (int rr = 0; rr < 4; ++rr) xv[rr] = xnext[rr];
+      }
+    }
+  } else {
+    if constexpr (FROM_XN) {
+      const int pt = threadIdx.x - 32 * B1_BASE_WARPS;
+      constexpr int NPT = 32 * B1_PROD_WARPS;
+      const int H0 = 4 * P.H4, W0 = 4 * P.W4;
+      const int XH = 4 * P.TQH + 9, XW = 4 * P.TQW + 9, AH = 4 * P.TQH + 7, AW = 4 * P.TQW + 7;
+      const int NPX = (2 * P.TQH + 3) * P.PW2;
+      const int XWP = P.XWP, AWP = P.AWP;
+      const int si = pt / P.PQW, sj = pt - si * P.PQW;
+      const bool s_ok = si < P.TQH && sj < P.TQW;
+      auto load_xn = [&](int tile, float* dst) {
+        const int b = (int)fdiv((unsigned)tile, P.div_img), rem = tile - b * tiles_img;
+        const int ty_ = (int)fdiv((unsigned)rem, P.div_x), tx_ = rem - ty_ * tiles_x;
+        const int gy0 = 4 * ty_ * P.TQH - 6, gx0 = 4 * tx_ * P.TQW - 6;
+        const float* xb = P.xn + (int64_t)b * H0 * W0;
+        for (int idx = pt; idx < XH * XW; idx += NPT) {
+          const int r = (int)fdiv((unsigned)idx, P.div_xw), c = idx - r * XW;
+          const int gy = gy0 + r, gx = gx0 + c;
+          const bool in = gy >= 0 && gy < H0 && gx >= 0 && gx < W0;
+          cp_async4(dst + (r * 2 + (c & 1)) * XWP + (c >> 1), in ? xb + (int64_t)gy * W0 + gx : P.xn, in);
+        }
+        cp_async_commit();
+      };
+      auto prod_sync = [] { asm volatile("bar.sync 1, %0;" ::"n"(NPT) : "memory"); };
+      const int xbuf = P.XB / 4;
+      if ((int)blockIdx.x < n_tiles) load_xn(blockIdx.x, sX);
+      uint32_t tcount = 0;
+      for (int tile = blockIdx.x; tile < n_tiles; tile += gridDim.x, ++tcount) {
+        const int b = (int)fdiv((unsigned)tile, P.div_img), rem = tile - b * tiles_img;
+        const int ty_ = (int)fdiv((unsigned)rem, P.div_x), tx_ = rem - ty_ * tiles_x;
+        const int qy0 = ty_ * P.TQH, qx0 = tx_ * P.TQW;
+        const float* X = sX + (tcount & 1) * xbuf;
+        cp_async_wait_all();
+        prod_sync();
+        if (pt < 128) {
+          const int k = tcount % B1_SKR;
+          tc::mbar_wait(&sk_empty[k], ((tcount / B1_SKR) & 1) ^ 1);
+          float skipv = 0.f;
+          if (s_ok) {
+            float sacc = 0.f;
+#pragma unroll
+            for (int rr = 0; rr < 4; ++rr) {
+              const float* row = X + (6 + 4 * si + rr) * 2 * XWP;
+#pragma unroll
+              for (int cc = 0; cc < 4; ++cc) sacc += row[(cc & 1) * XWP + 3 + 2 * sj + (cc >> 1)];
+            }
+            skipv = sacc * (1.0f / 16.0f);
+          }
+          sSk[k * 128 + pt] = skipv;
+          __syncwarp();
+          if (lane == 0) tc::mbar_arrive(&sk_full[k]);
+        }
+        const int ay0 = 4 * qy0 - 5, ax0 = 4 * qx0 - 5;
+        for (int idx = pt; idx < AH * 2 * AWP; idx += NPT) {
+          const int rp = (int)fdiv((unsigned)idx, P.div_awp), k = idx - rp * AWP;
+          const int r = rp >> 1, p = rp & 1, c = 2 * k + p;
+          if (c >= AW) continue;
+          float2 acc0 = make_float2(0.f, 0.f), acc1 = acc0;
+#pragma unroll
+          for (int ky = 0; ky < 3; ++ky) {
+            const float* row = X + (r + ky) * 2 * XWP + k;
+#pragma unroll
+            for (int kx = 0; kx < 3; ++kx) {
+              const float g = row[((p + kx) & 1) * XWP + ((p + kx) >> 1)];
+              const float* w = &P.sw.w0[(ky * 3 + kx) * 4];
+              acc0 = fma2(g, make_float2(w[0], w[1]), acc0);
+              acc1 = fma2(g, make_float2(w[2], w[3]), acc1);
+            }
+          }
+          const int gy = ay0 + r, gx = ax0 + c;
+          float4 v = make_float4(0.f, 0.f, 0.f, 0.f);
+          if (gy >= 0 && gy < H0 && gx >= 0 && gx < W0)
+            v = make_float4(fmaxf(acc0.x + P.sw.b0[0], 0.f), fmaxf(acc0.y + P.sw.b0[1], 0.f), fmaxf(acc1.x + P.sw.b0[2], 0.f),
+                            fmaxf(acc1.y + P.sw.b0[3], 0.f));
+          sA[idx] = v;
+        }
+        prod_sync();
+        if (tile + (int)gridDim.x < n_tiles) load_xn(tile + (int)gridDim.x, sX + ((tcount + 1) & 1) * xbuf);
+        const int s = tcount % B1_NP;
+        tc::mbar_wait(&p_empty[s], ((tcount / B1_NP) & 1) ^ 1);
+        unsigned char* pb = sP + (size_t)s * P.PB;
+        const int y20 = 2 * qy0 - 2, x20 = 2 * qx0 - 2;
+        auto a2_rows = [&](int px, auto HF) {
+          constexpr int hf = decltype(HF)::value;
+          const int ph = (int)fdiv((unsigned)px, P.div_pw2), pw = px - ph * P.PW2;
+          const int y = y20 + ph, x = x20 + pw;
+          uint2 hv = make_uint2(0u, 0u), lv = hv;
+          if (y >= 0 && y < H2 && x >= 0 && x < W2) {
+            float2 acc0 = make_float2(0.f, 0.f), acc1 = acc0;
+#pragma unroll
+            for (int ky = 0; ky < 3; ++ky)
+#pragma unroll
+              for (int kx = 0; kx < 3; ++kx) {
+                const float4 av = sA[((2 * ph + ky) * 2 + (kx & 1)) * AWP + pw + (kx >> 1)];
+                const float* w = &P.sw.w1[(ky * 3 + kx) * 32 + hf * 4];
+                acc0 = fma2(av.x, make_float2(w[0], w[1]), acc0);
+                acc1 = fma2(av.x, make_float2(w[2], w[3]), acc1);
+                acc0 = fma2(av.y, make_float2(w[8], w[9]), acc0);
+                acc1 = fma2(av.y, make_float2(w[10], w[11]), acc1);
+                acc0 = fma2(av.z, make_float2(w[16], w[17]), acc0);
+                acc1 = fma2(av.z, make_float2(w[18], w[19]), acc1);
+                acc0 = fma2(av.w, make_float2(w[24], w[25]), acc0);
+                acc1 = fma2(av.w, make_float2(w[26], w[27]), acc1);
+              }
+            const float* bb = &P.sw.b1[hf * 4];
+            const float v0 = fmaxf(acc0.x + bb[0], 0.f), v1 = fmaxf(acc0.y + bb[1], 0.f);
+            const float v2 = fmaxf(acc1.x + bb[2], 0.f), v3 = fmaxf(acc1.y + bb[3], 0.f);
+            const __half2 h01 = __floats2half2_rn(v0, v1), h23 = __floats2half2_rn(v2, v3);
+            const float2 f01 = __half22float2(h01), f23 = __half22float2(h23);
+            hv = make_uint2(half2_bits(h01), half2_bits(h23));
+            lv = make_uint2(half2_bits(__floats2half2_rn(v0 - f01.x, v1 - f01.y)), half2_bits(__floats2half2_rn(v2 - f23.x, v3 - f23.y)));
+          }
+          unsigned char* rp = pb + px * 32;
+          const int sw = (px >> 2) & 1;
+          *reinterpret_cast<uint2*>(rp + (sw << 4) + hf * 8) = hv;
+          *reinterpret_cast<uint2*>(rp + ((sw ^ 1) << 4) + hf * 8) = lv;
+        };
+        const int n_items = 2 * ((NPX + 31) & ~31);
+        for (int idx = pt; idx < n_items; idx += NPT) {
+          const int px = (idx >> 6) * 32 + (idx & 31);
+          if (px >= NPX) continue;
+          if ((idx >> 5) & 1) a2_rows(px, std::integral_constant<int, 1>());
+          else a2_rows(px, std::integral_constant<int, 0>());
+        }
+        tc::fence_proxy_async();
+        __syncwarp();
+        if (lane == 0) tc::mbar_arrive(&p_full[s]);
+      }
     }
   }
   tc::tc_fence_before();
@@ -282,10 +456,28 @@
   }
 }
 
-struct Block1Tile { int TQH, TQW, M2; };
-
-static Block1Tile pick_block1_tile(int H4, int W4) {
-  Block1Tile best = {0, 0, 0};
+struct Block1Geom {
+  int TQH, TQW, M2, PW2, PQW, PB, PLB, XWP, AWP, XB, AB;
+  size_t smem;
+};
+static Block1Geom block1_geom(int tqh, int tqw, bool from_xn) {
+  Block1Geom g;
+  g.TQH = tqh; g.TQW = tqw;
+  g.PW2 = 2 * tqw + 3;
+  g.PQW = tqw + 1;
+  g.M2 = cdiv((2 * tqh + 1) * g.PW2, 128);
+  g.PB = (int)align_up((size_t)(g.M2 * 128 + 2 * g.PW2 + 2) * 32, 1024);
+  g.PLB = (int)align_up((size_t)(128 + g.PQW + 1) * 32, 1024);
+  g.XWP = (4 * tqw + 10) / 2;
+  g.AWP = (4 * tqw + 8) / 2;
+  g.XB = from_xn ? (int)align_up((size_t)(4 * tqh + 9) * 2 * g.XWP * 4, 128) : 0;
+  g.AB = from_xn ? (4 * tqh + 7) * 2 * g.AWP * 16 : 0;
+  g.smem = 1024 + B1_W_PAD + (size_t)B1_NP * g.PB + (size_t)8 * g.PLB + 2 * (size_t)g.XB + g.AB + (from_xn ? B1_SKR * 512 : 0) + 1024;
+  return g;
+}
+
+static Block1Geom pick_block1_tile(int H4, int W4, bool from_xn) {
+  Block1Geom best = {};
   double best_cost = 1e30;
   for (int tqw = 4; tqw <= 62; ++tqw) {
     const int pqw = tqw + 1, pw2 = 2 * tqw + 3;
@@ -293,8 +485,13 @@
       const int m2 = cdiv((2 * tqh + 1) * pw2, 128);
       if ((m2 * 128 + 2 * pw2 + 2) * 32 > B1_PB_MAX || (128 + pqw + 1) * 32 > B1_PLANE_MAX) continue;
       const double tiles = (double)cdiv(W4, tqw) * cdiv(H4, tqh);
-      const double cost = tiles * ((m2 + 1) * 128.0 + 0.15 * (2 * tqh + 3) * pw2);
-      if (cost < best_cost) { best_cost = cost; best = {tqh, tqw, m2}; }
+      double cost = tiles * ((m2 + 1) * 128.0 + 0.15 * (2 * tqh + 3) * pw2);
+      if (from_xn) {
+        if (block1_geom(tqh, tqw, true).smem > (size_t)B1_SMEM_MAX) continue;
+        const double fma = (4.0 * tqh + 7) * (4 * tqw + 7) * 36 + (2.0 * tqh + 3) * pw2 * 288;
+        cost = fmax(3.5 * cost, tiles * fma / 90.0);
+      }
+      if (cost < best_cost) { best_cost = cost; best = block1_geom(tqh, tqw, from_xn); }
     }
   }
   return best;
@@ -307,6 +504,7 @@
   return g_block1_fused && !unfused;
 }
 
+template <bool FROM_XN>
 static int launch_block1_fused(const xfeat_ctx* ctx, const __half* a2_split, const float* xn, int B, int H4, int W4,
                                __half* out_split, float* out_f32, cudaStream_t st) {
   PFN_encodeTiled enc = get_encode_tiled();
@@ -314,27 +512,38 @@
     set_error("cuTensorMapEncodeTiled entry point not available");
     return XF_E_CUDA;
   }
-  const Block1Tile tl = pick_block1_tile(H4, W4);
+  const Block1Geom g = pick_block1_tile(H4, W4, FROM_XN);
+  XF_REQUIRE(g.TQH > 0, "block1_tc: no tile shape fits %d x %d", H4, W4);
   Block1Params P;
-  P.TQH = tl.TQH; P.TQW = tl.TQW; P.M2 = tl.M2;
-  P.PW2 = 2 * tl.TQW + 3;
-  P.PQW = tl.TQW + 1;
-  P.PB = (int)align_up((size_t)(tl.M2 * 128 + 2 * P.PW2 + 2) * 32, 1024);
-  P.PLB = (int)align_up((size_t)(128 + P.PQW + 1) * 32, 1024);
+  memset(&P, 0, sizeof(P));
+  P.TQH = g.TQH; P.TQW = g.TQW; P.M2 = g.M2;
+  P.PW2 = g.PW2;
+  P.PQW = g.PQW;
+  P.PB = g.PB;
+  P.PLB = g.PLB;
   int cols = 32;
-  while (cols < 2 * tl.M2 * 16 + 128) cols *= 2;
+  while (cols < 2 * g.M2 * 16 + 128) cols *= 2;
   P.tmem_cols = cols;
-  const int H2 = 2 * H4, W2 = 2 * W4;
-  const cuuint64_t dims[4] = {16, (cuuint64_t)W2, (cuuint64_t)H2, (cuuint64_t)B};
-  const cuuint64_t strides[3] = {32, (cuuint64_t)W2 * 32, (cuuint64_t)H2 * W2 * 32};
-  const cuuint32_t box[4] = {16, (cuuint32_t)P.PW2, (cuuint32_t)(2 * P.TQH + 3), 1};
-  const cuuint32_t estr[4] = {1, 1, 1, 1};
-  CUresult r = enc(&P.amap, CU_TENSOR_MAP_DATA_TYPE_FLOAT16, 4, (void*)a2_split, dims, strides, box, estr,
-                   CU_TENSOR_MAP_INTERLEAVE_NONE, CU_TENSOR_MAP_SWIZZLE_32B, CU_TENSOR_MAP_L2_PROMOTION_L2_256B,
-                   CU_TENSOR_MAP_FLOAT_OOB_FILL_NONE);
-  if (r != CUDA_SUCCESS) {
-    set_error("cuTensorMapEncodeTiled(block1 a2 patch) failed: %d", (int)r);
-    return XF_E_CUDA;
+  CUresult r;
+  if (!FROM_XN) {
+    const int H2 = 2 * H4, W2 = 2 * W4;
+    const cuuint64_t dims[4] = {16, (cuuint64_t)W2, (cuuint64_t)H2, (cuuint64_t)B};
+    const cuuint64_t strides[3] = {32, (cuuint64_t)W2 * 32, (cuuint64_t)H2 * W2 * 32};
+    const cuuint32_t box[4] = {16, (cuuint32_t)P.PW2, (cuuint32_t)(2 * P.TQH + 3), 1};
+    const cuuint32_t estr[4] = {1, 1, 1, 1};
+    r = enc(&P.amap, CU_TENSOR_MAP_DATA_TYPE_FLOAT16, 4, (void*)a2_split, dims, strides, box, estr, CU_TENSOR_MAP_INTERLEAVE_NONE,
+            CU_TENSOR_MAP_SWIZZLE_32B, CU_TENSOR_MAP_L2_PROMOTION_L2_256B, CU_TENSOR_MAP_FLOAT_OOB_FILL_NONE);
+    if (r != CUDA_SUCCESS) {
+      set_error("cuTensorMapEncodeTiled(block1 a2 patch) failed: %d", (int)r);
+      return XF_E_CUDA;
+    }
+  } else {
+    P.sw = stem01_weights(ctx->h_weights, ctx->table);
+    P.XB = g.XB; P.AB = g.AB;
+    P.XWP = g.XWP; P.AWP = g.AWP;
+    P.div_xw = make_fastdiv((unsigned)(4 * g.TQW + 9));
+    P.div_awp = make_fastdiv((unsigned)g.AWP);
+    P.div_pw2 = make_fastdiv((unsigned)g.PW2);
   }
   const int layers[2] = {L_B1_2, L_B1_3}, nrows[2] = {8, 32};
   CUtensorMap* maps[2] = {&P.w2map, &P.w3map};
@@ -365,23 +574,38 @@
   XF_REQUIRE(n_tiles < (1 << 22), "block1_tc: too many tiles (%d)", n_tiles);
   P.div_img = make_fastdiv((unsigned)tiles_img);
   P.div_x = make_fastdiv((unsigned)cdiv(W4, P.TQW));
-  const size_t smem = 1024 + B1_W_PAD + (size_t)B1_NP * P.PB + (size_t)8 * P.PLB + 1024;
   const int grid = n_tiles < ctx->sm_count ? n_tiles : ctx->sm_count;
-  XF_DYN_SMEM(block1_tc_kernel, smem);
-  block1_tc_kernel<<<grid, B1_THREADS, smem, st>>>(P);
+  XF_DYN_SMEM(block1_tc_kernel<FROM_XN>, g.smem);
+  block1_tc_kernel<FROM_XN><<<grid, b1_threads<FROM_XN>(), g.smem, st>>>(P);
   XF_LAUNCH_CHECK();
   return XF_OK;
 }
 
+static int require_block1_weights(const xfeat_ctx* ctx) {
+  XF_REQUIRE(ctx->d_tcw && ctx->tc_off[L_B1_2] != (size_t)-1 && ctx->tc_off[L_B1_3] != (size_t)-1,
+             "block1_tc: block1 weights not prepared for the tensor-core path");
+  return XF_OK;
+}
+
 int launch_block1_tail(const xfeat_ctx* ctx, const __half* a2_split, const float* xn, int B, int H4, int W4, __half* a3_split,
                        __half* out_split, float* out_f32, cudaStream_t st) {
-  XF_REQUIRE(ctx->d_tcw && ctx->tc_off[L_B1_2] != (size_t)-1 && ctx->tc_off[L_B1_3] != (size_t)-1,
-             "block1_tc: block1 weights not prepared for the tensor-core path");
+  if (int rc = require_block1_weights(ctx)) return rc;
   XF_REQUIRE(out_split || out_f32, "block1_tc: no output");
-  if (block1_fused()) return launch_block1_fused(ctx, a2_split, xn, B, H4, W4, out_split, out_f32, st);
+  if (block1_fused()) return launch_block1_fused<false>(ctx, a2_split, xn, B, H4, W4, out_split, out_f32, st);
   int rc = launch_conv_tc(ctx, L_B1_2, a2_split, B, 2 * H4, 2 * W4, a3_split, nullptr, st);
   if (rc) return rc;
   return launch_conv_tc(ctx, L_B1_3, a3_split, B, 2 * H4, 2 * W4, out_split, out_f32, st, xn);
+}
+
+int launch_block1(const xfeat_ctx* ctx, const float* xn, int B, int H4, int W4, __half* a2_split, __half* a3_split,
+                  __half* out_split, float* out_f32, cudaStream_t st) {
+  if (int rc = require_block1_weights(ctx)) return rc;
+  XF_REQUIRE(out_split || out_f32, "block1_tc: no output");
+  if (block1_fused() && stem_fused()) return launch_block1_fused<true>(ctx, nullptr, xn, B, H4, W4, out_split, out_f32, st);
+  int rc = launch_stem_chain(ctx->h_weights, ctx->table, xn, nullptr, (float*)a2_split, nullptr, nullptr, nullptr, B, 4 * H4, 4 * W4,
+                             st, 1);
+  if (rc) return rc;
+  return launch_block1_tail(ctx, a2_split, xn, B, H4, W4, a3_split, out_split, out_f32, st);
 }
 
 }
@@ -403,3 +627,15 @@
   if (rc) return rc;
   return xf::launch_block1_tail(ctx, a2s, d_xn, B, H / 4, W / 4, a2s + npix2 * 16, nullptr, d_x1s, st);
 }
+
+extern "C" int xfeat_debug_block1(xfeat_ctx* ctx, const float* d_xn, int B, int H, int W, float* d_x1s, void* d_scratch,
+                                  size_t scratch_bytes, void* stream) {
+  XF_REQUIRE(ctx && d_xn && d_x1s && d_scratch, "debug_block1: null pointer");
+  XF_REQUIRE(B > 0 && B <= 65535 && H > 0 && W > 0 && H % 4 == 0 && W % 4 == 0, "debug_block1: bad shape B=%d H=%d W=%d", B, H, W);
+  const int64_t npix2 = (int64_t)B * (H / 2) * (W / 2);
+  const int per_px = xf::block1_fused() ? 32 : 64;
+  XF_REQUIRE(scratch_bytes >= (size_t)npix2 * per_px, "debug_block1: scratch must hold B*(H/2)*(W/2)*%d bytes", per_px);
+  XF_CUDA(cudaSetDevice(ctx->device));
+  __half* a2s = (__half*)d_scratch;
+  return xf::launch_block1(ctx, d_xn, B, H / 4, W / 4, a2s, a2s + npix2 * 16, nullptr, d_x1s, (cudaStream_t)stream);
+}
diff --git a/accelerated_features_b200/csrc/common.cuh b/accelerated_features_b200/csrc/common.cuh
--- a/accelerated_features_b200/csrc/common.cuh
+++ b/accelerated_features_b200/csrc/common.cuh
@@ -115,6 +115,7 @@
         "l"(*reinterpret_cast<const unsigned long long*>(&c)));
   return r;
 }
+__device__ __forceinline__ float2 fma2(float a, float2 w, float2 c) { return f2_fma(make_float2(a, a), w, c); }
 __device__ __forceinline__ float2 f2_mul(float2 a, float2 b) {
   float2 r;
   asm("mul.rn.f32x2 %0, %1, %2;"
@@ -179,6 +180,16 @@
 int launch_unfold8_split(const float* xn, __half* out, int B, int Hc, int Wc, cudaStream_t st);
 int launch_stem_chain(const float* h_weights, const LayerTable& t, const float* xn, float* a1, float* a2, float* a3,
                       float* x1s, __half* x1s_split32, int B, int H, int W, cudaStream_t st, int tc_tail = 0);
+struct Stem01W {
+  float w0[9 * 4];
+  float b0[4];
+  float w1[9 * 4 * 8];
+  float b1[8];
+};
+Stem01W stem01_weights(const float* h_weights, const LayerTable& t);
+bool stem_fused();
+int launch_block1(const xfeat_ctx* ctx, const float* xn, int B, int H4, int W4, __half* a2_split, __half* a3_split,
+                  __half* out_split, float* out_f32, cudaStream_t st);
 int launch_fuse_pyramid(const float* x3, const float* x4, const float* x5, float* out, __half* out_split, int B, int H3,
                         int W3, cudaStream_t st);
 int launch_fuse_pyramid_split(const __half* x3, const __half* x4, const __half* x5, __half* out_split, int B, int H3, int W3,
diff --git a/accelerated_features_b200/csrc/stem.cu b/accelerated_features_b200/csrc/stem.cu
--- a/accelerated_features_b200/csrc/stem.cu
+++ b/accelerated_features_b200/csrc/stem.cu
@@ -97,23 +97,6 @@
         sp[g] = make_uint4(hw[0], hw[1], hw[2], hw[3]);
         sp[4 + g] = make_uint4(lw[0], lw[1], lw[2], lw[3]);
       }
-      return;
-    }
-  }
-  if constexpr (COUT == 8) {
-    if (out_split32 != nullptr) {
-      uint32_t hw[4], lw[4];
-#pragma unroll
-      for (int j = 0; j < 4; ++j) {
-        const __half2 h = __floats2half2_rn(res[2 * j], res[2 * j + 1]);
-        const float2 hf = __half22float2(h);
-        const __half2 l = __floats2half2_rn(res[2 * j] - hf.x, res[2 * j + 1] - hf.y);
-        hw[j] = *reinterpret_cast<const uint32_t*>(&h);
-        lw[j] = *reinterpret_cast<const uint32_t*>(&l);
-      }
-      uint4* sp = reinterpret_cast<uint4*>(out_split32 + (((int64_t)b * Ho + oy) * Wo + ox) * 16);
-      sp[0] = make_uint4(hw[0], hw[1], hw[2], hw[3]);
-      sp[1] = make_uint4(lw[0], lw[1], lw[2], lw[3]);
       return;
     }
   }
@@ -139,23 +122,6 @@
   return XF_OK;
 }
 
-struct Stem01W {
-  float w0[9 * 4];
-  float b0[4];
-  float w1[9 * 4 * 8];
-  float b1[8];
-};
-
-__device__ __forceinline__ float2 fma2(float a, float2 w, float2 c) {
-  float2 r;
-  const float2 aa = make_float2(a, a);
-  asm("fma.rn.f32x2 %0, %1, %2, %3;"
-      : "=l"(*reinterpret_cast<unsigned long long*>(&r))
-      : "l"(*reinterpret_cast<const unsigned long long*>(&aa)), "l"(*reinterpret_cast<const unsigned long long*>(&w)),
-        "l"(*reinterpret_cast<const unsigned long long*>(&c)));
-  return r;
-}
-
 __global__ void __launch_bounds__(128) stem01_kernel(const __grid_constant__ Stem01W P, const float* __restrict__ xn,
                                                      __half* __restrict__ out_split8, int H, int W) {
   const int Ho = H >> 1, Wo = W >> 1;
@@ -239,29 +205,37 @@
   }
 }
 
+Stem01W stem01_weights(const float* h_weights, const LayerTable& t) {
+  Stem01W P;
+  memcpy(P.w0, h_weights + t.w_off[L_B1_0], sizeof(P.w0));
+  memcpy(P.b0, h_weights + t.b_off[L_B1_0], sizeof(P.b0));
+  memcpy(P.w1, h_weights + t.w_off[L_B1_1], sizeof(P.w1));
+  memcpy(P.b1, h_weights + t.b_off[L_B1_1], sizeof(P.b1));
+  return P;
+}
+
 static int g_stem_fused = 1;
+
+bool stem_fused() {
+  static const bool unfused = getenv("XFEAT_STEM_UNFUSED") != nullptr;
+  return g_stem_fused && !unfused;
+}
 
 int launch_stem_chain(const float* h_weights, const LayerTable& t, const float* xn, float* a1, float* a2, float* a3,
                       float* x1s, __half* x1s_split32, int B, int H, int W, cudaStream_t st, int tc_tail) {
   const float* hw = h_weights;
   int rc;
-  static const bool unfused = getenv("XFEAT_STEM_UNFUSED") != nullptr;
-  if (tc_tail && g_stem_fused && !unfused) {
-    Stem01W P;
-    memcpy(P.w0, hw + t.w_off[L_B1_0], sizeof(P.w0));
-    memcpy(P.b0, hw + t.b_off[L_B1_0], sizeof(P.b0));
-    memcpy(P.w1, hw + t.w_off[L_B1_1], sizeof(P.w1));
-    memcpy(P.b1, hw + t.b_off[L_B1_1], sizeof(P.b1));
+  if (tc_tail) {
     dim3 grid(cdiv(W / 4, 32), cdiv(H / 4, 4), B);
-    stem01_kernel<<<grid, 128, 0, st>>>(P, xn, (__half*)a2, H, W);
+    stem01_kernel<<<grid, 128, 0, st>>>(stem01_weights(hw, t), xn, (__half*)a2, H, W);
     XF_LAUNCH_CHECK();
     return XF_OK;
   }
   rc = launch_stem<1, 4, 1, false>(hw + t.w_off[L_B1_0], hw + t.b_off[L_B1_0], nullptr, nullptr, xn, nullptr, a1, nullptr, B, H, W, st);
   if (rc) return rc;
-  rc = launch_stem<4, 8, 2, false>(hw + t.w_off[L_B1_1], hw + t.b_off[L_B1_1], nullptr, nullptr, a1, nullptr, a2,
-                                   tc_tail ? (__half*)a2 : nullptr, B, H, W, st);
-  if (rc || tc_tail) return rc;
+  rc = launch_stem<4, 8, 2, false>(hw + t.w_off[L_B1_1], hw + t.b_off[L_B1_1], nullptr, nullptr, a1, nullptr, a2, nullptr, B, H,
+                                   W, st);
+  if (rc) return rc;
   rc = launch_stem<8, 8, 1, false>(hw + t.w_off[L_B1_2], hw + t.b_off[L_B1_2], nullptr, nullptr, a2, nullptr, a3, nullptr, B, H / 2, W / 2, st);
   if (rc) return rc;
   rc = launch_stem<8, 24, 2, true>(hw + t.w_off[L_B1_3], hw + t.b_off[L_B1_3], hw + t.w_off[L_SKIP1], hw + t.b_off[L_SKIP1],
@@ -270,3 +244,6 @@
 }
 
 }
+
+extern "C" void xfeat_set_stem_fused(int on) { xf::g_stem_fused = on ? 1 : 0; }
+extern "C" int xfeat_get_stem_fused(void) { return xf::stem_fused() ? 1 : 0; }
diff --git a/include/xfeat_b200.h b/include/xfeat_b200.h
--- a/include/xfeat_b200.h
+++ b/include/xfeat_b200.h
@@ -56,6 +56,8 @@
 XF_API int xfeat_get_conv_impl(void);
 XF_API void xfeat_set_block1_fused(int on);
 XF_API int xfeat_get_block1_fused(void);
+XF_API void xfeat_set_stem_fused(int on);
+XF_API int xfeat_get_stem_fused(void);
 XF_API size_t xfeat_net_workspace_bytes(int B, int H, int W);
 XF_API int xfeat_net(xfeat_ctx* ctx, const float* d_xn, int B, int H, int W, float* d_feats, float* d_heat,
               float* d_reliability, float* d_kpt_logits, void* d_ws, size_t ws_bytes, void* stream);
@@ -141,6 +143,9 @@
 XF_API int xfeat_debug_block1_tail(xfeat_ctx* ctx, const float* d_a2, const float* d_xn, int B, int H, int W, float* d_x1s,
                                    void* d_scratch, size_t scratch_bytes, void* stream);
 
+XF_API int xfeat_debug_block1(xfeat_ctx* ctx, const float* d_xn, int B, int H, int W, float* d_x1s, void* d_scratch,
+                              size_t scratch_bytes, void* stream);
+
 #ifdef __cplusplus
 }
 #endif
```
